# mkln/spamtree

Hardware: AMD Instinct MI355X
Metric: Gibbs iterations/sec + achieved HBM GB/s, n=1e6 grid, 1/2/4/8 MI355X (higher is better)
Workload: dtype f64

## Files before the change

include/spamtree_hip.h:

```cpp
#ifndef SPAMTREE_HIP_H
#define SPAMTREE_HIP_H

#include <stdint.h>

#ifdef __cplusplus
extern "C" {
#endif

#define ST_OK 0
#define ST_ERR_CHOL_ROOT 1
#define ST_ERR_CHOL_REF 2
#define ST_ERR_CHOL_LEAF 3
#define ST_ERR_CHOL_SAMPLE_REF 10
#define ST_ERR_CHOL_SAMPLE_LEAF 11
#define ST_ERR_USAGE (-1)
#define ST_ERR_HIP (-2)
#define ST_ERR_TOPOLOGY (-3)
#define ST_ERR_UNSUPPORTED (-4)

#define ST_MAX_Q 6
#define ST_MAX_ANCESTORS 24

typedef struct st_handle_s *st_handle;

typedef struct st_problem {
  int64_t n_all;
  int32_t d;
  int32_t q;
  int32_t p;
  int32_t n_groups;
  int64_t n_blocks;
  const double *y;
  const double *X;
  const double *coords;
  const int64_t *mv_id;
  const int64_t *res_is_ref;
  const int64_t *block_names;
  const int64_t *block_groups;
  const int64_t *indexing_ptr;
  const int64_t *indexing_idx;
  const int64_t *parents_ptr;
  const int64_t *parents_idx;
  const int64_t *children_ptr;
  const int64_t *children_idx;
} st_problem;

typedef struct st_options {
  int32_t device;
  int32_t reference_quirks;
  int32_t rank;
  int32_t world;
  int32_t force_generic;
  int32_t reserved;
} st_options;

int st_create(const st_problem *pb, const st_options *opt, st_handle *out);
int st_destroy(st_handle h);
const char *st_last_error(st_handle h);

int st_set_w(st_handle h, const double *w);
int st_get_w(st_handle h, double *w);
int st_set_beta(st_handle h, const double *Bcoeff);
int st_set_tausq_inv(st_handle h, const double *tausq_inv);
int st_get_xb(st_handle h, double *xb);

int st_factor(st_handle h, int slot, const double *theta, int ntheta, double *loglik);
int st_factor_enqueue(st_handle h, int slot, const double *theta, int ntheta);
int st_factor_is_async(st_handle h);
int st_factor_finish(st_handle h, double *loglik);
int st_factor_begin(st_handle h, int slot, const double *theta, int ntheta);
int st_factor_ahead_levels(st_handle h);
int st_factor_ahead_enable(st_handle h, int enable);

int st_swap(st_handle h);

int st_sample_w(st_handle h, const double *z, uint64_t seed, uint32_t iter);

int st_loglik_w(st_handle h, int slot, double *loglik);

int st_sample_w_loglik(st_handle h, const double *z, uint64_t seed, uint32_t iter, int slot, double *loglik);
int st_sample_w_loglik_begin(st_handle h, const double *z, uint64_t seed, uint32_t iter, int slot);
int st_sample_w_loglik_end(st_handle h, double *loglik);

int st_predict(st_handle h, int theta_changed);

int st_beta_stats(st_handle h, double *xty);
int st_tausq_stats(st_handle h, double *ssq, int64_t *n_obs_by_q);
int st_xtx(st_handle h, double *xtx);

int st_yhat(st_handle h, const double *noise, uint64_t seed, uint32_t iter, double *yhat);

int st_block_dims(st_handle h, int64_t u, int64_t *m, int64_t *P, int32_t *is_ref, int32_t *n_obs);
int st_get_block(st_handle h, int slot, int64_t u, double *negRiH, double *Ri);
int st_get_comps(st_handle h, int slot, double *logdetCi_comps, double *loglik_w_comps);

int st_algorithmic_bytes(st_handle h, double *out5, double *flops3);
int st_probe_peaks(int device, int64_t bytes, int reps, double *out3);
int st_probe_math(int32_t fn, const double *x, int64_t n, int32_t device, double *out);
#define ST_N_KERNEL_FAMILIES 8
int st_profile_enable(st_handle h, int enable);
int st_profile_get(st_handle h, double *ms_total, int64_t *launches);
int st_profile_levels(st_handle h, int32_t *n_levels, double *ms_by_level, double *bytes_by_level, int32_t cap);
#define ST_KERNEL_GENERIC_LDS 0
#define ST_KERNEL_GENERIC_SCRATCH 1
#define ST_KERNEL_MFMA 2
#define ST_KERNEL_QUAD 3
#define ST_KERNEL_BIGMFMA 4
#define ST_KERNEL_WIDE 5
#define ST_KERNEL_LCHAIN 6
#define ST_KERNEL_LCHAIN_REF 7
int st_level_info(st_handle h, int32_t *n_levels, int32_t *kernel, int32_t *max_m, int32_t *max_P, int32_t *n_blocks, int32_t cap);
#define ST_ROUTE_NONE 0
#define ST_ROUTE_A_SLOTS 3
int st_route_info(st_handle h, int32_t *n_levels, int32_t *phase_a, int32_t *phase_b, int32_t *phase_p, int32_t cap);
const char *st_route_name(int32_t code);
int st_synchronize(st_handle h);
void *st_stream(st_handle h);

int st_cross_covariance_ag10(const double *coords1, const int64_t *mv1, int64_t n1, const double *coords2, const int64_t *mv2,
                             int64_t n2, const double *ai1, const double *ai2, const double *phi_i, const double *thetamv,
                             const double *Dmat, int32_t q, int32_t device, double *out);
int st_summary_reset(st_handle h);
int st_summary_accumulate(st_handle h, uint64_t seed, uint32_t iter);
int st_summary_get(st_handle h, double *w_mean, double *yhat_mean, int64_t *n_accumulated);
int st_summary_reserve(st_handle h, int64_t keep);
int st_summary_quantile(st_handle h, double q, double *w_q, double *yhat_q);

int st_points_set(st_handle h, int64_t n_new, const double *coords, const int64_t *mv, const int64_t *anchor, const double *X);
int st_points_predict(st_handle h, int mode, const double *z, uint64_t seed, uint32_t iter, double *w_new, double *cond_mean,
                      double *cond_var, double *yhat_new);
int st_points_info(st_handle h, int32_t *route, int64_t *n_groups, double *alg_bytes, double *flops);
const char *st_points_route_name(int32_t code);

int st_points_accumulate(st_handle h, uint64_t seed, uint32_t iter, double *w_new, double *cond_mean, double *cond_var, double *yhat_new);
int st_points_summary_reset(st_handle h);
int st_points_summary_reserve(st_handle h, int64_t keep);
int st_points_summary_get(st_handle h, double *mean, double *var, double *w_mean, double *yhat_mean, int64_t *n_accumulated);
int st_points_summary_quantile(st_handle h, double q, double *w_q, double *yhat_q);

int st_simulate(st_handle h, int nd, const double *z, const double *eps, uint64_t seed, uint32_t iter0, double *w_out, double *y_out);
int st_simulate_info(st_handle h, int nd, int32_t *route_mask, double *alg_bytes, double *flops);
const char *st_simulate_route_name(int32_t code);

int st_set_stream(st_handle h, void *stream);

int st_comm_unique_id(void *out, int32_t cap);
int st_comm_init(st_handle h, const void *unique_id);
int st_shard_plan(const st_problem *pb, int32_t world, int64_t *owner , int32_t *cut_level);
int st_shard_plan_opt(const st_problem *pb, const st_options *opt, int32_t world, int64_t *owner , int32_t *cut_level);
int st_shard_info(st_handle h, int32_t *rank, int32_t *world, int32_t *cut_level, int64_t *owned_blocks, int64_t *owned_rows);
int st_factor_local(st_handle h, int slot, const double *theta, int ntheta);
int st_loglik_local(st_handle h, int slot);
int st_mg_pack_comps(st_handle h, int slot, void **dev_ptr, int64_t *len);
int st_mg_finish(st_handle h, double *loglik);
int st_sample_w_local(st_handle h, const double *z, uint64_t seed, uint32_t iter);
int st_mg_top_region(st_handle h, void **dev_ptr, int64_t *len);
int st_sample_w_top(st_handle h);
int st_mg_pack_w(st_handle h, void **dev_ptr, int64_t *len);
int st_mg_unpack_w(st_handle h);
int st_mg_gather_w_pack(st_handle h, void **send_ptr, void **recv_ptr, int64_t *count_per_rank);
int st_mg_gather_w_unpack(st_handle h);
// ... 6 lines not shown
```

spamtree_amd/_lib.py:

```python
import ctypes as C
import os

HERE = os.path.dirname(os.path.abspath(__file__))
LIB_PATH = os.environ.get("SPAMTREE_LIB") or os.path.join(HERE, "libspamtree_hip.so")

c_dp = C.POINTER(C.c_double)
c_ip = C.POINTER(C.c_int64)


class StProblem(C.Structure):
    _fields_ = [("n_all", C.c_int64), ("d", C.c_int32), ("q", C.c_int32), ("p", C.c_int32), ("n_groups", C.c_int32),
                ("n_blocks", C.c_int64), ("y", c_dp), ("X", c_dp), ("coords", c_dp), ("mv_id", c_ip),
                ("res_is_ref", c_ip), ("block_names", c_ip), ("block_groups", c_ip), ("indexing_ptr", c_ip),
                ("indexing_idx", c_ip), ("parents_ptr", c_ip), ("parents_idx", c_ip), ("children_ptr", c_ip),
                ("children_idx", c_ip)]


class StOptions(C.Structure):
    _fields_ = [("device", C.c_int32), ("reference_quirks", C.c_int32), ("rank", C.c_int32), ("world", C.c_int32),
                ("force_generic", C.c_int32), ("reserved", C.c_int32)]


H = C.c_void_p
SIGNATURES = {
    "st_create": (C.c_int, [C.POINTER(StProblem), C.POINTER(StOptions), C.POINTER(H)]),
    "st_destroy": (C.c_int, [H]),
    "st_last_error": (C.c_char_p, [H]),
    "st_set_w": (C.c_int, [H, c_dp]),
    "st_get_w": (C.c_int, [H, c_dp]),
    "st_set_beta": (C.c_int, [H, c_dp]),
    "st_set_tausq_inv": (C.c_int, [H, c_dp]),
    "st_get_xb": (C.c_int, [H, c_dp]),
    "st_factor": (C.c_int, [H, C.c_int, c_dp, C.c_int, c_dp]),
    "st_factor_begin": (C.c_int, [H, C.c_int, c_dp, C.c_int]),
    "st_factor_ahead_levels": (C.c_int, [H]),
    "st_swap": (C.c_int, [H]),
    "st_sample_w": (C.c_int, [H, c_dp, C.c_uint64, C.c_uint32]),
    "st_loglik_w": (C.c_int, [H, C.c_int, c_dp]),
    "st_sample_w_loglik": (C.c_int, [H, c_dp, C.c_uint64, C.c_uint32, C.c_int, c_dp]),
    "st_sample_w_loglik_begin": (C.c_int, [H, c_dp, C.c_uint64, C.c_uint32, C.c_int]),
    "st_sample_w_loglik_end": (C.c_int, [H, c_dp]),
    "st_predict": (C.c_int, [H, C.c_int]),
    "st_beta_stats": (C.c_int, [H, c_dp]),
    "st_tausq_stats": (C.c_int, [H, c_dp, c_ip]),
    "st_xtx": (C.c_int, [H, c_dp]),
    "st_yhat": (C.c_int, [H, c_dp, C.c_uint64, C.c_uint32, c_dp]),
    "st_block_dims": (C.c_int, [H, C.c_int64, c_ip, c_ip, C.POINTER(C.c_int32), C.POINTER(C.c_int32)]),
    "st_get_block": (C.c_int, [H, C.c_int, C.c_int64, c_dp, c_dp]),
    "st_get_comps": (C.c_int, [H, C.c_int, c_dp, c_dp]),
    "st_algorithmic_bytes": (C.c_int, [H, c_dp, c_dp]),
    "st_factor_ahead_enable": (C.c_int, [H, C.c_int]),
    "st_probe_peaks": (C.c_int, [C.c_int, C.c_int64, C.c_int, c_dp]),
    "st_probe_math": (C.c_int, [C.c_int32, c_dp, C.c_int64, C.c_int32, c_dp]),
    "st_profile_enable": (C.c_int, [H, C.c_int]),
    "st_profile_get": (C.c_int, [H, c_dp, c_ip]),
    "st_profile_levels": (C.c_int, [H, C.POINTER(C.c_int32), c_dp, c_dp, C.c_int32]),
    "st_level_info": (C.c_int, [H, C.POINTER(C.c_int32), C.POINTER(C.c_int32), C.POINTER(C.c_int32), C.POINTER(C.c_int32),
                                C.POINTER(C.c_int32), C.c_int32]),
    "st_route_info": (C.c_int, [H, C.POINTER(C.c_int32), C.POINTER(C.c_int32), C.POINTER(C.c_int32), C.POINTER(C.c_int32),
                                C.c_int32]),
    "st_route_name": (C.c_char_p, [C.c_int32]),
    "st_synchronize": (C.c_int, [H]),
    "st_stream": (C.c_void_p, [H]),
    "st_set_stream": (C.c_int, [H, C.c_void_p]),
    "st_shard_plan": (C.c_int, [C.POINTER(StProblem), C.c_int32, c_ip, C.POINTER(C.c_int32)]),
    "st_shard_plan_opt": (C.c_int, [C.POINTER(StProblem), C.POINTER(StOptions), C.c_int32, c_ip, C.POINTER(C.c_int32)]),
    "st_shard_info": (C.c_int, [H, C.POINTER(C.c_int32), C.POINTER(C.c_int32), C.POINTER(C.c_int32), c_ip, c_ip]),
    "st_factor_local": (C.c_int, [H, C.c_int, c_dp, C.c_int]),
    "st_factor_enqueue": (C.c_int, [H, C.c_int, c_dp, C.c_int]),
    "st_factor_finish": (C.c_int, [H, c_dp]),
    "st_factor_is_async": (C.c_int, [H]),
    "st_loglik_local": (C.c_int, [H, C.c_int]),
    "st_mg_pack_comps": (C.c_int, [H, C.c_int, C.POINTER(C.c_void_p), c_ip]),
    "st_mg_finish": (C.c_int, [H, c_dp]),
    "st_sample_w_local": (C.c_int, [H, c_dp, C.c_uint64, C.c_uint32]),
    "st_mg_top_region": (C.c_int, [H, C.POINTER(C.c_void_p), c_ip]),
    "st_sample_w_top": (C.c_int, [H]),
    "st_mg_pack_w": (C.c_int, [H, C.POINTER(C.c_void_p), c_ip]),
    "st_mg_unpack_w": (C.c_int, [H]),
    "st_mg_gather_w_pack": (C.c_int, [H, C.POINTER(C.c_void_p), C.POINTER(C.c_void_p), c_ip]),
    "st_mg_gather_w_unpack": (C.c_int, [H]),
    "st_cross_covariance_ag10": (C.c_int, [c_dp, c_ip, C.c_int64, c_dp, c_ip, C.c_int64, c_dp, c_dp, c_dp, c_dp, c_dp, C.c_int32,
                                           C.c_int32, c_dp]),
    "st_summary_reset": (C.c_int, [H]),
    "st_summary_accumulate": (C.c_int, [H, C.c_uint64, C.c_uint32]),
    "st_summary_get": (C.c_int, [H, c_dp, c_dp, c_ip]),
    "st_summary_reserve": (C.c_int, [H, C.c_int64]),
    "st_summary_quantile": (C.c_int, [H, C.c_double, c_dp, c_dp]),
    "st_comm_unique_id": (C.c_int, [C.c_void_p, C.c_int32]),
    "st_comm_init": (C.c_int, [H, C.c_void_p]),
    "st_points_set": (C.c_int, [H, C.c_int64, c_dp, c_ip, c_ip, c_dp]),
    "st_points_predict": (C.c_int, [H, C.c_int, c_dp, C.c_uint64, C.c_uint32, c_dp, c_dp, c_dp, c_dp]),
    "st_points_info": (C.c_int, [H, C.POINTER(C.c_int32), c_ip, c_dp, c_dp]),
    "st_points_route_name": (C.c_char_p, [C.c_int32]),
    "st_points_accumulate": (C.c_int, [H, C.c_uint64, C.c_uint32, c_dp, c_dp, c_dp, c_dp]),
    "st_points_summary_reset": (C.c_int, [H]),
    "st_points_summary_reserve": (C.c_int, [H, C.c_int64]),
    "st_points_summary_get": (C.c_int, [H, c_dp, c_dp, c_dp, c_dp, c_ip]),
    "st_points_summary_quantile": (C.c_int, [H, C.c_double, c_dp, c_dp]),
    "st_simulate": (C.c_int, [H, C.c_int, c_dp, c_dp, C.c_uint64, C.c_uint32, c_dp, c_dp]),
    "st_simulate_info": (C.c_int, [H, C.c_int, C.POINTER(C.c_int32), c_dp, c_dp]),
    "st_simulate_route_name": (C.c_char_p, [C.c_int32]),
}


class StmFlags(C.Structure):
    _fields_ = [("adapting", C.c_int32), ("sample_beta", C.c_int32), ("sample_tausq", C.c_int32),
                ("sample_theta", C.c_int32), ("sample_w", C.c_int32), ("sample_predicts", C.c_int32)]


SIGNATURES.update({
    "stm_create": (C.c_int, [C.POINTER(StProblem), C.POINTER(StOptions), c_dp, c_dp, c_dp, C.c_int, c_dp, C.c_double,
                             C.c_uint64, C.POINTER(StmFlags), C.POINTER(H)]),
    "stm_init": (C.c_int, [H]),
    "stm_destroy": (C.c_int, [H]),
    "stm_last_error": (C.c_char_p, [H]),
    "stm_handle": (C.c_void_p, [H]),
    "stm_step": (C.c_int, [H, C.c_int]),
    "stm_state": (C.c_int, [H, c_dp, c_dp, c_dp, c_dp, c_dp, c_ip, c_dp]),
    "spamtree_mv_mcmc_c": (C.c_int, [C.POINTER(StProblem), C.POINTER(StOptions), c_dp, c_dp, C.c_int, c_dp, C.c_double,
                                     c_dp, C.c_int, C.c_int, C.c_int, C.c_uint64, C.POINTER(StmFlags), c_dp, c_dp,
# ... 33 lines not shown
```

spamtree_amd/csrc/misc_kernels.hpp:

```cpp
#pragma once
#include "st_device.hpp"

struct LoglikArgs {
  const Blk *blks;
  const int *anc_idx;
  const int *list;
  int nlist;
  const double *panels;
  const double *w;
  double *loglik_c;
  int maxP, maxM;
};

struct LoglikGrpArgs {
  const Blk *blks;
  const int *anc_idx;
  const Grp *grps;
  const int *list;
  int nlist;
  const double *panels;
  const double *w;
  double *loglik_c;
  int maxP;
  const long long *gdesc;
  int gd_stride;
};

#define SUM2_WG 64
#define STATS_WG 1024
struct QtArgs {
  const double *draws;
  long long n;
  int keep, Kpad, R;
  double q;
  double *out;
};

#ifdef ST_DEFS_MISC
__global__ void k_normals(double *z, const long long *dev2model, long long n, unsigned iter, unsigned stream, unsigned long long seed) {
  const long long i = (long long)blockIdx.x * blockDim.x + threadIdx.x;
  if (i < n) z[i] = philox_normal((unsigned long long)dev2model[i], iter, stream, seed);
}


__global__ __launch_bounds__(NT) void k_loglik(LoglikArgs A) {
  extern __shared__ double lds[];
  __shared__ int s_am[MAXJ], s_ao[MAXJ + 1];
  __shared__ long long s_arow[MAXJ];
  __shared__ double s_red[NT / 64];
  const int tid = threadIdx.x, lane = tid & 63, wid = tid >> 6;
  double *wv = lds;
  double *tv = wv + (A.maxP + A.maxM);
  for (int li = blockIdx.x; li < A.nlist; li += gridDim.x) {
    const int b = A.list[li];
    const Blk B = A.blks[b];
    const int m = B.m, P = B.P, J = B.nanc, ld = B.ld;
    __syncthreads();
    if (tid < J) {
      const int a = A.anc_idx[B.anc_ptr + tid];
      s_am[tid] = A.blks[a].m;
      s_arow[tid] = A.blks[a].row0;
    }
    __syncthreads();
    if (tid == 0) {
      int o = 0;
      for (int t = 0; t < J; ++t) { s_ao[t] = o; o += s_am[t]; }
      s_ao[J] = o;
    }
    __syncthreads();
    for (int t = 0; t < J; ++t)
      for (int i = tid; i < s_am[t]; i += NT) wv[s_ao[t] + i] = A.w[s_arow[t] + i];
    for (int i = tid; i < m; i += NT) wv[P + i] = A.w[B.row0 + i];
    __syncthreads();
    const double *N = A.panels + B.panel_off;
    for (int i = wid; i < m; i += NT / 64) {
      double acc = 0.0;
      for (int k = lane; k < P; k += 64) acc += N[(size_t)i * ld + k] * wv[k];
      acc = wave_sum(acc);
      if (lane == 0) tv[i] = acc;
    }
    __syncthreads();
    double part = 0.0;
    for (int i = tid; i < m; i += NT) {
      double acc = tv[i];
      if (B.isref) {
        for (int j = 0; j <= i; ++j) acc += N[(size_t)i * ld + P + j] * wv[P + j];
      } else {
        acc += N[(size_t)i * ld + P] * wv[P + i];
      }
      part += acc * acc;
    }
    const double wcore = block_sum(part, s_red);
    if (tid == 0) A.loglik_c[b] = (double)m * HL2PI - 0.5 * wcore;
  }
}


__global__ __launch_bounds__(NT, 8) void k_loglik_grp(LoglikGrpArgs A) {
  extern __shared__ double lds[];
  __shared__ int s_am[MAXJ], s_ao[MAXJ + 1];
  __shared__ long long s_arow[MAXJ];
  __shared__ long long s_bpan[32], s_brow[32];
  __shared__ int s_bld[32], s_cb[32];
  __shared__ double s_e2[32];
  __shared__ long long s_gd[GD_MAXW];
  const int tid = threadIdx.x, lane = tid & 63, wid = tid >> 6;
  double *wv = lds;
  {
    const long long *gd = A.gdesc + (size_t)A.list[blockIdx.x] * A.gd_stride;
    for (int i = tid; i < A.gd_stride; i += NT) s_gd[i] = gd[i];
  }
  __syncthreads();
  const GdHead B0 = gd_unpack(s_gd, tid, s_am, s_ao, s_arow, nullptr, nullptr, s_bpan, s_brow, s_bld, nullptr);
  const Grp G = {B0.row0, B0.blk0, B0.nblk, B0.M, B0.P};
  const int M = G.M, P = G.P, J = B0.nanc;
  const bool refgrp = B0.isref != 0;
  if (tid >= 128 && tid < 128 + 32) wv[P + tid - 128] = (tid - 128 < M) ? A.w[G.row0 + tid - 128] : 0.0;
  if (tid >= 32 && tid < 64) {
    const int j = tid - 32;
    int bi = 0;
    if (j < M) { const long long r = G.row0 + j; while (bi + 1 < G.nblk && r >= s_gd[8 + 4 * J + 3 * (bi + 1) + 1]) ++bi; }
    s_cb[j] = bi;
  }
  __syncthreads();
  const int rowlen = P + (refgrp ? M : 1);
#pragma unroll 1
  for (int b = 0; b < 2; ++b) {
    double v[4][5];
#pragma unroll
    for (int rr = 0; rr < 4; ++rr) {
      const int j = wid + 4 * (4 * b + rr), jc = min(j, M - 1);
      const int bi = s_cb[jc];
      const double *src = A.panels + s_bpan[bi] + (size_t)(G.row0 + jc - s_brow[bi]) * s_bld[bi];
#pragma unroll
      for (int c = 0; c < 5; ++c) {
        const int k = lane + 64 * c;
        v[rr][c] = (j < M && k < rowlen) ? src[k] : 0.0;
      }
    }
    if (b == 0) {
      for (int k = tid; k < P; k += NT) {
        int t = 0;
        while (t + 1 < J && k >= s_ao[t + 1]) ++t;
        wv[k] = A.w[s_arow[t] + (k - s_ao[t])];
      }
      __syncthreads();
    }
#pragma unroll
    for (int rr = 0; rr < 4; ++rr) {
      const int j = wid + 4 * (4 * b + rr);
      double acc = 0.0;
#pragma unroll
      for (int c = 0; c < 5; ++c) {
        const int k = lane + 64 * c;
        const double wk = k < P ? wv[k] : (refgrp ? (k < rowlen ? wv[k] : 0.0) : wv[P + min(j, 31)]);
        acc += v[rr][c] * wk;
      }
      acc = wave_sum(acc);
      if (lane == 0 && j < 32) s_e2[j] = acc * acc;
    }
  }
  __syncthreads();
  if (tid < G.nblk) {
    double wc = 0.0;
    int cnt = 0;
    for (int j = 0; j < M; ++j)
      if (s_cb[j] == tid) { wc += s_e2[j]; ++cnt; }
    A.loglik_c[G.blk0 + tid] = (double)cnt * HL2PI - 0.5 * wc;
  }
}

__global__ __launch_bounds__(NT) void k_sum2_partial(const double *a, const double *b, int n, double *partial) {
  __shared__ double sa[NT], sb[NT];
  const int chunk = (n + SUM2_WG - 1) / SUM2_WG;
  const int lo = blockIdx.x * chunk, hi = min(n, lo + chunk);
  double xa = 0.0, xb = 0.0;
  for (int i = lo + threadIdx.x; i < hi; i += NT) { xa += a[i]; xb += b[i]; }
  sa[threadIdx.x] = xa; sb[threadIdx.x] = xb;
  __syncthreads();
  for (int s2 = NT / 2; s2 > 0; s2 >>= 1) {
    if ((int)threadIdx.x < s2) { sa[threadIdx.x] += sa[threadIdx.x + s2]; sb[threadIdx.x] += sb[threadIdx.x + s2]; }
    __syncthreads();
  }
  if (threadIdx.x == 0) { partial[2 * blockIdx.x] = sa[0]; partial[2 * blockIdx.x + 1] = sb[0]; }
}
__global__ void k_sum2_final(const double *partial, double *out) {
  if (threadIdx.x < 2) {
    double s2 = 0.0;
    for (int g = 0; g < SUM2_WG; ++g) s2 += partial[2 * g + threadIdx.x];
    out[threadIdx.x] = s2;
  }
}

__global__ void k_xb(const double *X, const int *mv, const double *B, long long n, int p, double *xb) {
  const long long i = (long long)blockIdx.x * blockDim.x + threadIdx.x;
  if (i >= n) return;
  const double *bj = B + (size_t)p * mv[i];
  double acc = 0.0;
  for (int j = 0; j < p; ++j) acc += X[(size_t)j * n + i] * bj[j];
  xb[i] = acc;
}

__global__ __launch_bounds__(NT) void k_stats(const double *X, const double *y, const double *w, const double *xb, const int *mv,
                                               const unsigned char *obs, const long long *partner, long long n, int p, int q,
                                               double *partial) {
  __shared__ double s_red[NT / 64];
  const int nq = p * q + q;
  double acc[QMAX * 8 + QMAX];
  for (int k = 0; k < nq; ++k) acc[k] = 0.0;
  const long long chunk = (n + gridDim.x - 1) / gridDim.x;
  const long long lo = (long long)blockIdx.x * chunk, hi = min(n, lo + chunk);
  for (long long i = lo + threadIdx.x; i < hi; i += NT) {
    if (!obs[i]) continue;
    const int v = mv[i];
    const double rw = y[i] - w[partner[i]];
    for (int j = 0; j < p; ++j) acc[v * p + j] += X[(size_t)j * n + i] * rw;
    const double e = y[i] - xb[i] - w[i];
    acc[p * q + v] += e * e;
  }
  for (int k = 0; k < nq; ++k) {
    const double s = block_sum(acc[k], s_red);
    if (threadIdx.x == 0) partial[(size_t)blockIdx.x * nq + k] = s;
  }
}
__global__ __launch_bounds__(NT) void k_stats_final(const double *partial, int nwg, int nq, double *out) {
  __shared__ double sm[NT];
  const int k = blockIdx.x;
  double s = 0.0;
  for (int g = threadIdx.x; g < nwg; g += NT) s += partial[(size_t)g * nq + k];
  sm[threadIdx.x] = s;
  __syncthreads();
  for (int o = NT / 2; o > 0; o >>= 1) {
    if ((int)threadIdx.x < o) sm[threadIdx.x] += sm[threadIdx.x + o];
    __syncthreads();
  }
  if (threadIdx.x == 0) out[k] = sm[0];
}

__global__ void k_yhat(const double *xb, const double *w, const double *noise, const int *mv, long long n, const double *tsq_inv_q,
                       double *yhat) {
  const long long i = (long long)blockIdx.x * blockDim.x + threadIdx.x;
  if (i < n) yhat[i] = xb[i] + w[i] + noise[i] / sqrt(tsq_inv_q[mv[i]]);
// ... 125 lines not shown
```

spamtree_amd/csrc/sample_kernels.hpp:

```cpp
#pragma once
#include "st_device.hpp"

struct SampleArgs {
  const Blk *blks;
  const int *anc_idx;
  const int *dch_idx;
  const int *list;
  int nlist;
  const double *panels;
  double *w;
  const double *y, *xb, *z;
  const int *mv;
  const unsigned char *obs;
  double *acc;
  int *errflag;
  double *scratch;
  long long scratch_stride;
  int maxP, maxM, maxLd;
  int do_gram;
  int no_fwd;
  int lds_sq;
  double *s0;
  const long long *s0off;
  double tausq_inv[QMAX];
};

struct GramBigArgs {
  const Blk *blks;
  const int *anc_idx, *dch_idx;
  const int *list;
  int nlist;
  const double *panels;
  double *acc;
  double *s0;
  const long long *s0off;
  int no_fwd;
  int mirror;
};

struct SampleFastArgs {
  const Blk *blks;
  const int *anc_idx, *dch_idx;
  const Grp *grps;
  int ngrp;
  const double *panels;
  double *w;
  const double *y, *xb, *z;
  const int *mv;
  double *acc;
  int *errflag;
  const long long *gdesc;
  int gd_stride;
  int ldN, Mr4, Mrows, maxP, av_dbl;
  int do_gram;
  int no_fwd;
  double tausq_inv[QMAX];
  const long long *gdesc_all;
  double *s0;
  const long long *s0off;
  int s0_mode;
};
#define GRAM_DIRECT_MAXCH 4

#ifdef ST_DEFS_SAMPLE

__device__ __forceinline__ void wave_chol_solve_lds(double *S, int ms, double *lcol, double *bv, const double *zg, int m, int *fail, int lane) {
  const int i0 = lane, i1 = 64 + (lane & 15), g1 = lane >> 4;
  const bool r0 = i0 < m, r1 = i1 < m;
  const bool two = m > 64;
  double c0 = r0 ? bv[i0] : 0.0, c1 = r1 ? bv[i1] : 0.0;
  double dr0 = 1.0, dr1 = 1.0;
  bool bad = false;
  for (int j = lane; j < m + 8; j += 64) lcol[j] = 0.0;
  for (int k = 0; k < m; ++k) {
    const double d = S[(size_t)k * ms + k];
    bad = bad || !(d > 0.0);
    double rp = __builtin_amdgcn_rsq(d);
    rp = rp * fma(-0.5 * d * rp, rp, 1.5);
    rp = rp * fma(-0.5 * d * rp, rp, 1.5);
    const bool u0 = r0 && i0 > k, u1 = r1 && i1 > k;
    const double l0 = u0 ? S[(size_t)i0 * ms + k] * rp : 0.0;
    const double l1 = u1 ? S[(size_t)i1 * ms + k] * rp : 0.0;
    const double ck = readlane_f64(k < 64 ? c0 : c1, k & 63);
    const double yk = ck * rp;
    c0 = (i0 == k) ? yk : fma(-l0, yk, c0);
    c1 = (i1 == k) ? yk : fma(-l1, yk, c1);
    dr0 = (i0 == k) ? rp : dr0;
    dr1 = (i1 == k) ? rp : dr1;
    if (u0) { S[(size_t)i0 * ms + k] = l0; lcol[i0] = l0; }
    if (u1 && g1 == 0) { S[(size_t)i1 * ms + k] = l1; lcol[i1] = l1; }
    __builtin_amdgcn_fence(__ATOMIC_ACQ_REL, "wavefront");
    if (r0) {
      double *row = S + (size_t)i0 * ms;
      for (int j0 = k + 1; j0 < m; j0 += 8) {
        double lj[8], a0[8];
#pragma unroll
        for (int q = 0; q < 8; ++q) lj[q] = lcol[j0 + q];
#pragma unroll
        for (int q = 0; q < 8; ++q) a0[q] = row[j0 + q];
#pragma unroll
        for (int q = 0; q < 8; ++q) row[j0 + q] = fma(-l0, lj[q], a0[q]);
      }
    }
    if (two) {
      if (r1) {
        double *row = S + (size_t)i1 * ms;
        for (int j0 = k + 1 + 8 * g1; j0 < m; j0 += 32) {
          double lj[8], a1[8];
#pragma unroll
          for (int q = 0; q < 8; ++q) lj[q] = lcol[j0 + q];
#pragma unroll
          for (int q = 0; q < 8; ++q) a1[q] = row[j0 + q];
#pragma unroll
          for (int q = 0; q < 8; ++q) row[j0 + q] = fma(-l1, lj[q], a1[q]);
        }
      }
    }
    __builtin_amdgcn_fence(__ATOMIC_ACQ_REL, "wavefront");
  }
  if (bad && lane == 0) *fail = 1;
  double t0 = r0 ? c0 + zg[i0] : 0.0, t1 = r1 ? c1 + zg[i1] : 0.0;
  for (int k = m - 1; k >= 0; --k) {
    const double wk = readlane_f64(k < 64 ? t0 : t1, k & 63) * readlane_f64(k < 64 ? dr0 : dr1, k & 63);
    t0 = (i0 == k) ? wk : ((r0 && i0 < k) ? fma(-S[(size_t)k * ms + i0], wk, t0) : t0);
    if (two) t1 = (i1 == k) ? wk : ((r1 && i1 < k) ? fma(-S[(size_t)k * ms + i1], wk, t1) : t1);
  }
  if (r0) bv[i0] = t0;
  if (r1 && g1 == 0) bv[i1] = t1;
}


template <bool BIG, bool NOREF = false>
__global__ __launch_bounds__(NT) void k_sample(SampleArgs A) {
  extern __shared__ double lds[];
  __shared__ int s_am[MAXJ], s_ao[MAXJ + 1];
  __shared__ long long s_arow[MAXJ], s_aoff[MAXJ + 1];
  __shared__ int s_fail;
  __shared__ long long s_choff[16];

  const int tid = threadIdx.x, lane = tid & 63, wid = tid >> 6;
  const int maxP = A.maxP, maxM = A.maxM;
  double *wv = lds;
  double *tv = wv + (maxP + maxM);
// ... 801 lines not shown
    const int t = u >> 1, it = u & 1;
    const bool self = t == J;
    const int ma = self ? M : s_am[t], oa = self ? P : s_ao[t];
    if (it * 16 >= ma) continue;
    const bool wide = ma > 16;
    auto chains = [&](const long long *rowoff, int Mr, d4 (&cq)[2]) __attribute__((always_inline)) {
      const int ns = (Mr + 3) >> 2;
      double b0[8], b1[8];
#pragma unroll
      for (int st = 0; st < 8; ++st) {
        const int r = 4 * st + l4;
        const bool rok = st < ns && r < Mr;
        const double *row = A.panels + rowoff[min(r, 31)] + oa + l15;
        b0[st] = rok ? row[0] : 0.0;
        b1[st] = (rok && wide) ? row[16] : 0.0;
      }
      cq[0] = (d4){0.0, 0.0, 0.0, 0.0}; cq[1] = cq[0];
#pragma unroll
      for (int st = 0; st < 8; ++st)
        if (st < ns) {
          const double ai = it ? b1[st] : b0[st];
          cq[0] = __builtin_amdgcn_mfma_f64_16x16x4f64(ai, b0[st], cq[0], 0, 0, 0);
          if (wide) cq[1] = __builtin_amdgcn_mfma_f64_16x16x4f64(ai, b1[st], cq[1], 0, 0, 0);
        }
    };
    auto store = [&](double *out, const d4 (&v)[2]) __attribute__((always_inline)) {
#pragma unroll
      for (int jt = 0; jt < 2; ++jt) {
        if (jt > 0 && !wide) continue;
#pragma unroll
        for (int r = 0; r < 4; ++r) {
          const int i = it * 16 + l4 + 4 * r, j = jt * 16 + l15;
          if (i < ma && j < ma) out[i * ma + j] = v[jt][r];
        }
      }
    };
    d4 chv[2];
    chv[0] = (d4){0.0, 0.0, 0.0, 0.0}; chv[1] = chv[0];
    for (int cc = 0; cc < nch; ++cc) {
      d4 cch[2];
      chains(s_crow[cc], s_cM[cc], cch);
#pragma unroll
      for (int q = 0; q < 2; ++q)
#pragma unroll
        for (int r = 0; r < 4; ++r) { cch[q][r] += 0.0; chv[q][r] += cch[q][r]; }
      if (self) store(A.acc + s_coff[cc] + B0.acc_len, cch);
    }
    if (!self) {
      d4 c[2];
      chains(s_rowoff, M, c);
#pragma unroll
      for (int q = 0; q < 2; ++q)
#pragma unroll
        for (int r = 0; r < 4; ++r) c[q][r] += chv[q][r];
      store(rec + s_aoff[t], c);
    }
  }
}

template <bool LAT>
__global__ __launch_bounds__(NT, LAT ? 2 : 5) void k_sample_lean(SampleFastArgs A) {
  extern __shared__ double lds[];
  __shared__ int s_am[MAXJ], s_ao[MAXJ + 1];
  __shared__ long long s_arow[MAXJ], s_aoff[MAXJ + 1];
  __shared__ long long s_bpan[32], s_brow[32], s_rowoff[32];
  __shared__ int s_bld[32], s_cb[32];
  __shared__ int s_fail;
  __shared__ long long s_coff[64];
  __shared__ int s_nch;
  __shared__ long long s_gd[GD_MAXW];

  const int tid = threadIdx.x;
  double *wv = lds;
  double *seg = wv + A.maxP + 32;
  double *tv = seg + A.av_dbl + 16, *ev = tv + 32, *bv = ev + 32, *tsq = bv + 32, *yx = tsq + 32, *zc = yx + 32, *rjv = zc + 32;
  double *Rc = rjv + 32;
  double *S = Rc + 32 * CH_LD;

  int gidx = blockIdx.x;
  {
    const int per = A.ngrp >> 3;
    if (gidx < per * 8) gidx = (gidx & 7) * per + (gidx >> 3);
  }
  for (int i = tid; i < A.gd_stride; i += NT) s_gd[i] = A.gdesc[(size_t)gidx * A.gd_stride + i];
  __syncthreads();
  const GdHead B0 = gd_unpack(s_gd, tid, s_am, s_ao, s_arow, nullptr, s_aoff, s_bpan, s_brow, s_bld, s_coff);
  const Grp G = {B0.row0, B0.blk0, B0.nblk, B0.M, B0.P};
  const int M = G.M, P = G.P, J = B0.nanc;
  const bool refgrp = B0.isref != 0;
  if (tid == 0) { s_fail = 0; s_nch = B0.ndch; }
  const long long so = (refgrp && A.s0off && A.s0_mode) ? A.s0off[B0.blk0] : -1;
  const bool s0_load = so >= 0 && A.s0_mode == 2;
  double xq[28], x2[28], ch2[4], s0v[3], smv[4];
  const int k2 = tid - 64;
  const int nch2 = A.no_fwd ? 0 : B0.ndch;
  if constexpr (LAT) {
    double t_ = 0.0, y_ = 0.0, xb_ = 0.0, z_ = 0.0, r_ = 0.0;
    int mv_ = 0;
    const bool rowthr = tid >= 32 && tid < 64 && tid - 32 < M;
    if (tid >= 32 && tid < 64) {
      const int j = tid - 32;
      int bi = 0;
      long long ro = 0;
      if (j < M) {
        const long long r = G.row0 + j;
        mv_ = A.mv[r]; y_ = A.y[r]; xb_ = A.xb[r]; z_ = A.z[r];
        const long long *gb = s_gd + 8 + 4 * J;
        while (bi + 1 < G.nblk && r >= gb[3 * (bi + 1) + 1]) ++bi;
        ro = gb[3 * bi] + (r - gb[3 * bi + 1]) * gb[3 * bi + 2];
        if (!refgrp) r_ = A.panels[ro + P];
      }
      s_cb[j] = bi; s_rowoff[j] = ro;
    }
    lds_barrier();
    double wreg = 0.0;
    int wk = -1;
    if (tid < P) {
      int t = 0;
      while (t + 1 < J && tid >= s_ao[t + 1]) ++t;
      wk = tid; wreg = A.w[s_arow[t] + (tid - s_ao[t])];
    }
    double rireg[3];
#pragma unroll
    for (int e = 0; e < 3; ++e) {
      const int idx = tid + NT * e, i = idx / M, j = idx - i * M;
      rireg[e] = (refgrp && idx < M * M && j <= i) ? A.panels[s_rowoff[i] + P + j] : 0.0;
    }
    {
      const int idx = tid, mj = M * J;
      const int ii = mj > 0 ? min(idx, mj - 1) : 0, r = J ? ii / J : 0, t = J ? ii - r * J : 0;
      const int ma = J ? s_am[t] : 0;
      const double *row = A.panels + s_rowoff[r] + (J ? s_ao[t] : 0);
#pragma unroll
      for (int jj = 0; jj < 28; ++jj) xq[jj] = (idx < mj && jj < ma) ? row[jj] : 0.0;
    }
#pragma unroll
    for (int cc = 0; cc < 4; ++cc)
      smv[cc] = (refgrp && tid < M && cc < B0.ndch) ? A.acc[s_coff[min(cc, max(B0.ndch - 1, 0))] + B0.acc_len + M * M + tid] : 0.0;
    if (k2 >= 0 && k2 < P) {
      int t = 0;
      while (t + 1 < J && k2 >= s_ao[t + 1]) ++t;
      const int ma = s_am[t], i = k2 - s_ao[t];
#pragma unroll
      for (int cc = 0; cc < 4; ++cc) ch2[cc] = (cc < nch2) ? A.acc[s_coff[min(cc, max(nch2 - 1, 0))] + s_aoff[t] + ma * ma + i] : 0.0;
#pragma unroll
      for (int rr = 0; rr < 28; ++rr) x2[rr] = (rr < M) ? A.panels[s_rowoff[min(rr, M - 1)] + k2] : 0.0;
    }
#pragma unroll
    for (int e = 0; e < 3; ++e) {
      const int idx = tid + NT * e, i = idx / M, j = idx - i * M;
      s0v[e] = (s0_load && idx < M * M && j <= i) ? A.s0[so + idx] : 0.0;
    }
    if (rowthr) t_ = A.tausq_inv[mv_];
    if (tid >= 32 && tid < 64) { const int j = tid - 32; tsq[j] = t_; yx[j] = y_ - xb_; zc[j] = z_; rjv[j] = r_; }
    if (wk >= 0) wv[wk] = wreg;
    for (int k = NT + tid; k < P; k += NT) {
      int t = 0;
      while (t + 1 < J && k >= s_ao[t + 1]) ++t;
      wv[k] = A.w[s_arow[t] + (k - s_ao[t])];
    }
    if (refgrp) {
#pragma unroll
      for (int e = 0; e < 3; ++e) {
        const int idx = tid + NT * e, i = idx / M, j = idx - i * M;
        if (idx < M * M) Rc[i * CH_LD + j] = rireg[e];
      }
      for (int idx = 3 * NT + tid; idx < M * M; idx += NT) {
        const int i = idx / M, j = idx - i * M;
        Rc[i * CH_LD + j] = (j <= i) ? A.panels[s_rowoff[i] + P + j] : 0.0;
      }
    }
    __syncthreads();
  } else {
  if (tid >= 32 && tid < 64) {
    const int j = tid - 32;
    double t_ = 0.0, y_ = 0.0, z_ = 0.0, r_ = 0.0;
    int bi = 0;
    long long ro = 0;
    if (j < M) {
      const long long r = G.row0 + j;
      t_ = A.tausq_inv[A.mv[r]]; y_ = A.y[r] - A.xb[r]; z_ = A.z[r];
      const long long *gb = s_gd + 8 + 4 * J;
      while (bi + 1 < G.nblk && r >= gb[3 * (bi + 1) + 1]) ++bi;
      ro = gb[3 * bi] + (r - gb[3 * bi + 1]) * gb[3 * bi + 2];
      if (!refgrp) r_ = A.panels[ro + P];
    }
    tsq[j] = t_; yx[j] = y_; zc[j] = z_; rjv[j] = r_; s_cb[j] = bi; s_rowoff[j] = ro;
  }
  __syncthreads();
  for (int k = tid; k < P; k += NT) {
    int t = 0;
    while (t + 1 < J && k >= s_ao[t + 1]) ++t;
    wv[k] = A.w[s_arow[t] + (k - s_ao[t])];
  }
  if (refgrp) {
    for (int idx = tid; idx < M * M; idx += NT) {
      const int i = idx / M, j = idx - i * M;
      Rc[i * CH_LD + j] = (j <= i) ? A.panels[s_rowoff[i] + P + j] : 0.0;
    }
  }
  __syncthreads();
  }
  for (int idx = tid; idx < M * J; idx += NT) {
    const int r = idx / J, t = idx - r * J;
    const int ma = s_am[t], oa = s_ao[t];
    const double *row = A.panels + s_rowoff[r] + oa;
    const double *wa = wv + oa;
    double a = 0.0;
    if (LAT && idx == tid && ma <= 28) {
#pragma unroll
      for (int jj = 0; jj < 28; ++jj) a += xq[jj] * ((jj < ma) ? wa[jj] : 0.0);
    } else
    for (int j0 = 0; j0 < ma; j0 += 16) {
      double x[16];
#pragma unroll
      for (int jj = 0; jj < 16; ++jj) x[jj] = (j0 + jj < ma) ? row[j0 + jj] : 0.0;
#pragma unroll
      for (int jj = 0; jj < 16; ++jj) a += x[jj] * ((j0 + jj < ma) ? wa[j0 + jj] : 0.0);
    }
    seg[t * 32 + r] = a;
  }
  __syncthreads();
  if (tid < M) {
    double a = 0.0;
    for (int t = 0; t < J; ++t) a += seg[t * 32 + tid];
    tv[tid] = a;
  }
  __syncthreads();
  if (refgrp) {
    for (int idx = tid; idx < M * M; idx += NT) {
      const int i = idx / M, j = idx - i * M;
      double a = 0.0;
      if (j <= i) {
        if (s0_load) a = (LAT && idx < 3 * NT) ? (idx < NT ? s0v[0] : (idx < 2 * NT ? s0v[1] : s0v[2])) : A.s0[so + idx];
        else {
          double ch[4];
          for (int c0 = 0; c0 < s_nch; c0 += 4) {
#pragma unroll
            for (int cc = 0; cc < 4; ++cc) ch[cc] = (c0 + cc < s_nch) ? A.acc[s_coff[min(c0 + cc, s_nch - 1)] + B0.acc_len + idx] : 0.0;
            if (c0 == 0) for (int k = i; k < M; ++k) a += Rc[k * CH_LD + i] * Rc[k * CH_LD + j];
#pragma unroll
            for (int cc = 0; cc < 4; ++cc) a += ch[cc];
          }
          if (s_nch == 0) for (int k = i; k < M; ++k) a += Rc[k * CH_LD + i] * Rc[k * CH_LD + j];
          if (so >= 0) A.s0[so + idx] = a;
        }
        if (i == j) a += tsq[i];
      }
      S[i * CH_LD + j] = a;
    }
    if (tid < M) {
      const int i = tid;
      double a = 0.0;
      for (int k = i; k < M; ++k) a -= Rc[k * CH_LD + i] * tv[k];
      double ch[4];
      for (int c0 = 0; c0 < s_nch; c0 += 4) {
#pragma unroll
        for (int cc = 0; cc < 4; ++cc)
          ch[cc] = (LAT && c0 == 0) ? smv[cc] : ((c0 + cc < s_nch) ? A.acc[s_coff[min(c0 + cc, s_nch - 1)] + B0.acc_len + M * M + i] : 0.0);
#pragma unroll
        for (int cc = 0; cc < 4; ++cc) a += ch[cc];
      }
      bv[i] = a + tsq[i] * yx[i];
    }
    double *pub = seg + 32 * J;
    if (M <= 27) {
      __syncthreads();
      if (tid < 64) wave_chol_solve<27>(S, bv, zc, wv + P, M, &s_fail, tid);
      __syncthreads();
    } else {
      team_chol_eliminate<5, NT>(S, S, M, M, pub, &s_fail, tid);
      if (tid < M) {
        double a = zc[tid];
        for (int j = 0; j <= tid; ++j) a += S[tid * CH_LD + j] * bv[j];
        ev[tid] = a;
      }
      __syncthreads();
      if (tid < M) {
        double a = 0.0;
        for (int i = tid; i < M; ++i) a += S[i * CH_LD + tid] * ev[i];
        wv[P + tid] = a;
      }
      __syncthreads();
    }
    if (tid < M) {
      const int i = tid;
      A.w[G.row0 + i] = wv[P + i];
      double a = tv[i];
      for (int j = 0; j <= i; ++j) a += Rc[i * CH_LD + j] * wv[P + j];
      ev[i] = a;
    }
  } else {
    if (tid < M) {
      const int j = tid;
      const double rj = rjv[j];
      const double sig = rj * rj + tsq[j];
      if (!(sig > 0.0)) s_fail = 1;
      const double mu = -rj * tv[j] + tsq[j] * yx[j];
      const double c = 1.0 / sqrt(sig);
      const double wj = c * c * mu + c * zc[j];
      A.w[G.row0 + j] = wj;
      ev[j] = rj * wj + tv[j];
    }
  }
  __syncthreads();
  for (int idx = tid; idx < J * 32; idx += NT) {
    const int r = idx & 31;
    seg[idx] = (r < M) ? ev[r] - seg[idx] : 0.0;
  }
  __syncthreads();
  double *rec = A.acc + B0.acc_off;
  const int kfirst = LAT ? (tid >= 64 ? k2 : NT - 64 + tid) : tid;
  for (int k = kfirst; k < P; k += NT) {
    int t = 0;
    while (t + 1 < J && k >= s_ao[t + 1]) ++t;
    const int ma = s_am[t], i = k - s_ao[t];
    const double *avt = seg + t * 32;
    const bool held = LAT && tid >= 64 && k == k2 && M <= 28;
    double ch[4];
    const int nch = A.no_fwd ? 0 : s_nch;
#pragma unroll
    for (int cc = 0; cc < 4; ++cc) ch[cc] = held ? ch2[cc] : ((cc < nch) ? A.acc[s_coff[min(cc, max(nch - 1, 0))] + s_aoff[t] + ma * ma + i] : 0.0);
    double a = 0.0;
    if (held) {
#pragma unroll
      for (int rr = 0; rr < 28; ++rr) a -= x2[rr] * avt[min(rr, 31)];
    } else
    for (int r0 = 0; r0 < M; r0 += 8) {
      double x[8];
#pragma unroll
      for (int rr = 0; rr < 8; ++rr) x[rr] = (r0 + rr < M) ? A.panels[s_rowoff[min(r0 + rr, M - 1)] + k] : 0.0;
#pragma unroll
      for (int rr = 0; rr < 8; ++rr) a -= x[rr] * avt[min(r0 + rr, 31)];
    }
#pragma unroll
    for (int cc = 0; cc < 4; ++cc) a += ch[cc];
    for (int c0 = 4; c0 < nch; c0 += 4) {
#pragma unroll
      for (int cc = 0; cc < 4; ++cc) ch[cc] = (c0 + cc < nch) ? A.acc[s_coff[min(c0 + cc, nch - 1)] + s_aoff[t] + ma * ma + i] : 0.0;
#pragma unroll
      for (int cc = 0; cc < 4; ++cc) a += ch[cc];
    }
    rec[s_aoff[t] + ma * ma + i] = a;
  }
  if (tid == 0 && s_fail) atomicMin(A.errflag, B0.level * 16 + (refgrp ? 10 : 11));
}
template __global__ void k_sample_lean<false>(SampleFastArgs);
template __global__ void k_sample_lean<true>(SampleFastArgs);

#define WSYNC() asm volatile("s_waitcnt lgkmcnt(0)" ::: "memory")
__global__ __launch_bounds__(NT, 3) void k_sample_wave(SampleFastArgs A) {
  extern __shared__ double lds[];
  __shared__ int s_failw[NT / 64];
  const int tid = threadIdx.x, lane = tid & 63, wid = tid >> 6;
  const int gidx = blockIdx.x * (NT / 64) + wid;
  if (gidx >= A.ngrp) return;
  double *base = lds + (size_t)wid * A.ldN;
  long long *s_gd = (long long *)base;
  double *wv = base + A.gd_stride;
  double *seg = wv + A.maxP + 32;
  double *tv = seg + A.av_dbl, *ev = tv + 32;
  double *Rc = ev + 32;
  if (lane == 0) s_failw[wid] = 0;
  for (int i = lane; i < A.gd_stride; i += 64) s_gd[i] = A.gdesc[(size_t)gidx * A.gd_stride + i];
  WSYNC();
  auto slo = [](long long v) { return __builtin_amdgcn_readfirstlane((int)(v & 0xffffffffLL)); };
  auto shi = [](long long v) { return __builtin_amdgcn_readfirstlane((int)(v >> 32)); };
  auto sll = [&](long long v) { return ((long long)shi(v) << 32) | (unsigned int)slo(v); };
  const long long row0 = sll(s_gd[0]), acc_off = sll(s_gd[1]);
  const int M = slo(s_gd[2]), P = shi(s_gd[2]), J = slo(s_gd[3]), level = shi(s_gd[4]);
  const int nch = slo(s_gd[5]), acc_len = shi(s_gd[5]);
  const long long *gb = s_gd + 8 + 4 * J;
  const long long bpan = sll(gb[0]);
  const int bld = (int)sll(gb[2]);
  const long long *coff = gb + 3;
  auto am_of = [&](int t) { return (int)(s_gd[8 + 4 * t] & 0xffffffffLL); };
  auto ao_of = [&](int t) { return (int)(s_gd[8 + 4 * t] >> 32); };
  const bool row = lane < M;
  const int li = min(lane, 31);
  double tsq = 0.0, yx = 0.0, zc = 0.0;
  if (row) { const long long r = row0 + lane; tsq = A.tausq_inv[A.mv[r]]; yx = A.y[r] - A.xb[r]; zc = A.z[r]; }
  for (int k = lane; k < P; k += 64) {
    int t = 0;
    for (int j = 1; j < J; ++j) t += k >= ao_of(j) ? 1 : 0;
    wv[k] = A.w[s_gd[8 + 4 * t + 1] + (k - ao_of(t))];
  }
  const int PS = P | 1;
  const int RG = min(4, (A.Mrows * CH_LD) / PS);
  if (RG >= 1) {
    constexpr int NRI = (27 * 27 + 63) / 64;
    double rireg[NRI];
#pragma unroll
    for (int q = 0; q < NRI; ++q) {
      const int idx = lane + 64 * q, i = idx / M, j = idx - i * M;
      rireg[q] = (idx < M * M && j <= i) ? A.panels[bpan + (size_t)i * bld + P + j] : 0.0;
    }
    double *stg = Rc;
    for (int r0 = 0; r0 < M; r0 += RG) {
      for (int c0 = 0; 64 * c0 < P; c0 += 4) {
        double x[4][4];
#pragma unroll
        for (int rr = 0; rr < 4; ++rr)
#pragma unroll
          for (int c = 0; c < 4; ++c) {
            const int k = lane + 64 * (c0 + c);
            x[rr][c] = (rr < RG && r0 + rr < M && k < P) ? A.panels[bpan + (size_t)(r0 + rr) * bld + k] : 0.0;
          }
#pragma unroll
        for (int rr = 0; rr < 4; ++rr)
#pragma unroll
          for (int c = 0; c < 4; ++c) {
            const int k = lane + 64 * (c0 + c);
            if (rr < RG && k < P) stg[rr * PS + k] = x[rr][c];
          }
      }
      WSYNC();
      if (lane < RG * J) {
        const int rr = lane / J, t = lane - rr * J, r = r0 + rr;
        if (r < M) {
          const int ma = am_of(t), oa = ao_of(t);
          const double *srow = stg + rr * PS + oa;
          const double *wa = wv + oa;
          double a = 0.0;
          for (int j = 0; j < ma; ++j) a += srow[j] * wa[j];
          seg[t * 32 + r] = a;
        }
      }
    }
    WSYNC();
#pragma unroll
    for (int q = 0; q < NRI; ++q) {
      const int idx = lane + 64 * q, i = idx / M, j = idx - i * M;
      if (idx < M * M) Rc[i * CH_LD + j] = rireg[q];
    }
    WSYNC();
  } else {
  for (int idx = lane; idx < M * M; idx += 64) {
    const int i = idx / M, j = idx - i * M;
    Rc[i * CH_LD + j] = (j <= i) ? A.panels[bpan + (size_t)i * bld + P + j] : 0.0;
  }
  WSYNC();
  for (int idx = lane; idx < M * J; idx += 64) {
    const int r = idx / J, t = idx - r * J;
    const int ma = am_of(t), oa = ao_of(t);
    const double *prow = A.panels + bpan + (size_t)r * bld + oa;
    const double *wa = wv + oa;
    double a = 0.0;
    for (int j0 = 0; j0 < ma; j0 += 16) {
      double x[16];
#pragma unroll
      for (int jj = 0; jj < 16; ++jj) x[jj] = (j0 + jj < ma) ? prow[j0 + jj] : 0.0;
#pragma unroll
      for (int jj = 0; jj < 16; ++jj) a += x[jj] * ((j0 + jj < ma) ? wa[j0 + jj] : 0.0);
    }
    seg[t * 32 + r] = a;
  }
  WSYNC();
  }
  double tvi = 0.0;
  if (row) { for (int t = 0; t < J; ++t) tvi += seg[t * 32 + lane]; tv[lane] = tvi; }
  WSYNC();
  double a[27];
#pragma unroll
  for (int j = 0; j < 27; ++j) a[j] = 0.0;
  double bv = 0.0;
  const long long so = (A.s0off && A.s0_mode) ? A.s0off[slo(s_gd[6])] : -1;
  if (so >= 0 && A.s0_mode == 2) {
    const double *sp = A.s0 + so + (size_t)li * M;
#pragma unroll
    for (int j = 0; j < 27; ++j) a[j] = (row && j <= lane) ? sp[j] : 0.0;
    for (int k = 0; k < M; ++k) bv -= Rc[k * CH_LD + li] * tv[k];
    for (int c = 0; c < nch; ++c) bv += row ? A.acc[coff[c] + acc_len + M * M + li] : 0.0;
  } else {
    for (int k = 0; k < M; ++k) {
      const double rk = Rc[k * CH_LD + li];
      bv -= rk * tv[k];
#pragma unroll
      for (int j = 0; j < 27; ++j) a[j] += rk * Rc[k * CH_LD + j];
    }
    for (int c = 0; c < nch; ++c) {
      const double *rc = A.acc + coff[c] + acc_len;
      double ch[27];
#pragma unroll
      for (int j = 0; j < 27; ++j) ch[j] = (row && j <= lane) ? rc[li * M + j] : 0.0;
      const double cv = row ? rc[M * M + li] : 0.0;
#pragma unroll
      for (int j = 0; j < 27; ++j) a[j] += ch[j];
      bv += cv;
    }
    if (so >= 0 && row) {
      double *sp = A.s0 + so + (size_t)li * M;
#pragma unroll
      for (int j = 0; j < 27; ++j) if (j <= lane) sp[j] = a[j];
    }
  }
#pragma unroll
  for (int j = 0; j < 27; ++j) {
    if (j == lane) a[j] += tsq;
    a[j] = (row && j <= lane) ? a[j] : (j == lane ? 1.0 : 0.0);
  }
  bv = row ? bv + tsq * yx : 0.0;
  const double wnew = wave_chol_solve_core<27>(a, bv, zc, M, &s_failw[wid], lane);
  if (row) { A.w[row0 + lane] = wnew; wv[P + lane] = wnew; }
  WSYNC();
  if (row) {
    double e = tvi;
    for (int j = 0; j <= lane; ++j) e += Rc[lane * CH_LD + j] * wv[P + j];
    ev[lane] = e;
  }
  WSYNC();
  for (int idx = lane; idx < J * 32; idx += 64) {
    const int r = idx & 31;
    seg[idx] = (r < M) ? ev[r] - seg[idx] : 0.0;
  }
  WSYNC();
  double *rec = A.acc + acc_off;
  const int nfw = A.no_fwd ? 0 : nch;
  for (int k = lane; k < P; k += 64) {
    int t = 0;
    for (int j = 1; j < J; ++j) t += k >= ao_of(j) ? 1 : 0;
    const int ma = am_of(t), i = k - ao_of(t);
    const long long aoff = s_gd[8 + 4 * t + 3];
    const double *avt = seg + t * 32;
    double ch[4];
#pragma unroll
    for (int cc = 0; cc < 4; ++cc) ch[cc] = (cc < nfw) ? A.acc[coff[min(cc, max(nfw - 1, 0))] + aoff + ma * ma + i] : 0.0;
    double acc = 0.0;
    for (int r0 = 0; r0 < M; r0 += 8) {
      double x[8];
#pragma unroll
      for (int rr = 0; rr < 8; ++rr) x[rr] = (r0 + rr < M) ? A.panels[bpan + (size_t)min(r0 + rr, M - 1) * bld + k] : 0.0;
#pragma unroll
      for (int rr = 0; rr < 8; ++rr) acc -= x[rr] * avt[min(r0 + rr, 31)];
    }
#pragma unroll
    for (int cc = 0; cc < 4; ++cc) acc += ch[cc];
// ... 368 lines not shown
```

spamtree_amd/csrc/spamtree_hip.hip:

```cpp

#include "st_device.hpp"
#include "factor_generic.hpp"
#include "factor_mfma.hpp"
#include "chol_blocked.hpp"
#include "factor_quad.hpp"
#include "factor_big.hpp"
#include "factor_wide.hpp"
#include "factor_lchain.hpp"
#include "sample_kernels.hpp"
#include "misc_kernels.hpp"
#include "predict_points.hpp"
#include "simulate_kernels.hpp"

static thread_local std::string g_create_error;
struct st_handle_s;
static void points_free(st_handle_s *h);

template <typename T>
struct DevBuf {
  T *p = nullptr;
  size_t n = 0;
  hipError_t alloc(size_t count) {
    n = count;
    if (count == 0) { p = nullptr; return hipSuccess; }
    return hipMalloc((void **)&p, count * sizeof(T));
  }
  hipError_t upload(const std::vector<T> &v) {
    hipError_t e = alloc(v.size());
    if (e != hipSuccess || v.empty()) return e;
    return hipMemcpy(p, v.data(), v.size() * sizeof(T), hipMemcpyHostToDevice);
  }
  void free() { if (p) (void)hipFree(p); p = nullptr; n = 0; }
};

struct LevelInfo {
  int first = 0, count = 0;
  int isref = 1;
  int maxP = 0, maxM = 0, maxMa = 0, maxLd = 0;
  bool big_factor = false, big_sample = false, sample_sq = false;
  size_t lds_factor = 0, lds_sample = 0, lds_loglik = 0;
  double alg_bytes_A = 0, alg_bytes_B = 0, alg_bytes_C = 0, alg_bytes_msg = 0;
  double flops_A = 0, flops_B = 0, flops_C = 0;
  bool fast = false;
  int grp_first = 0, grp_count = 0, Pm4 = 0, ldKV = 2, ldS = 2, SRm = 1, stage_dbl = 0;
  size_t lds_fast = 0;
  int ldN = 2, Mr4 = 4, Mrows = 1, av_dbl = 224, maxJ = 0;
  size_t lds_sfast = 0, lds_slean = 0;
  bool bigmfma = false;
  int wide_first = 0, wide_count = 0, wide_maxN = 0;
  size_t lds_wide = 0;
  int bm_ldS = 0;
  size_t lds_bigmfma = 0;
  int lchain = 0;
  bool lchain_ref = false;
  size_t lds_ref_finish = 0;
  int rf_first = 0;
  int lc_first = 0, lc_count = 0;
  int quad_first = 0, quad_count = 0, qown_lo = 0, qown_n = 0, q_ldS = 0, q_nkx = 0;
  long long vl_off = -1;
  size_t lds_quad = 0;
  int own_lo = 0, own_n = 0, gown_lo = 0, gown_n = 0;
};

enum RouteCode : int {
  R_NONE = ST_ROUTE_NONE,
  R_MARGINAL_INVCHOL_WAVE, R_MARGINAL_INVCHOL,
  R_FACTOR_LDS, R_FACTOR_SCRATCH, R_PREDICT_LDS, R_PREDICT_SCRATCH,
  R_QUAD32_REF_WCH, R_QUAD32_REF, R_QUAD32_LEAF, R_QUAD38_REF_WCH, R_QUAD38_REF, R_QUAD38_LEAF,
  R_QUAD44_REF_WCH, R_QUAD44_REF, R_QUAD44_LEAF, R_QUAD50_REF_WCH, R_QUAD50_REF, R_QUAD50_LEAF,
  R_FACTOR_MFMA, R_LCHAIN96, R_LCHAIN136, R_REF_FINISH, R_LCHAIN_SCALARS, R_FACTOR_WIDE, R_BIGMFMA3, R_BIGMFMA4, R_BIGMFMA5,
  R_GRAM, R_GRAM_DIRECT, R_GRAM_BIG,
  R_SAMPLE_MFMA, R_LEAF_SEG4, R_LEAF_SEG6, R_SAMPLE_LEAF, R_SAMPLE_WAVE, R_SAMPLE_LEAN_LAT, R_SAMPLE_LEAN,
  R_SAMPLE_BIG_REF, R_SAMPLE_LEAF_WIDE, R_SAMPLE_BIG_LEAF, R_SAMPLE_SMALL,
  R_COUNT
};
static const char *const k_route_names[R_COUNT] = {
  "",
  "k_marginal_invchol_wave", "k_marginal_invchol",
  "k_factor<false, MODE_FACTOR>", "k_factor<true, MODE_FACTOR>", "k_factor<false, MODE_PREDICT>", "k_factor<true, MODE_PREDICT>",
  "k_factor_quad<4, 32, 8, true, true>", "k_factor_quad<4, 32, 8, true, false>", "k_factor_quad<4, 32, 8, false, true>",
  "k_factor_quad<4, 38, 10, true, true>", "k_factor_quad<4, 38, 10, true, false>", "k_factor_quad<4, 38, 10, false, true>",
  "k_factor_quad<4, 44, 11, true, true>", "k_factor_quad<4, 44, 11, true, false>", "k_factor_quad<4, 44, 11, false, true>",
  "k_factor_quad<4, 50, 13, true, true>", "k_factor_quad<4, 50, 13, true, false>", "k_factor_quad<4, 50, 13, false, true>",
  "k_factor_mfma", "k_factor_lchain<96>", "k_factor_lchain<136>", "k_factor_ref_finish", "k_lchain_scalars", "k_factor_wide<WG_JT>",
  "k_factor_bigmfma<3, 5, 34>", "k_factor_bigmfma<4, 5, 34>", "k_factor_bigmfma<5, 3, 24>",
  "k_gram", "k_gram_direct", "k_gram_big",
  "k_sample_mfma", "k_sample_leaf_seg<4>", "k_sample_leaf_seg<6>", "k_sample_leaf", "k_sample_wave", "k_sample_lean<true>",
  "k_sample_lean<false>", "k_sample<true, false>", "k_sample_leaf_wide", "k_sample<true, true>", "k_sample<false>",
};

struct Switches {
  int wide = 1, split_gram = 1, sample_wave = 1;
  bool lchain = true, lchain_ref = true, gram_big = true, gram_direct = true, sample_lean = true, sample_lat = true,
       leaf_seg = true, leaf_wide = true, async_top = true;
  int lchain_ref_min = 1;
  int factor_gen = 3;
  int quad_units = 0;
  int quad_min = -1;
};

static Switches read_switches() {
  auto level = [](const char *name) {
    const char *e = getenv(name);
    return (e && e[0] == '0') ? 0 : ((e && e[0] == '2') ? 2 : 1);
  };
  Switches s;
  s.wide = level("SPAMTREE_WIDE"); s.split_gram = level("SPAMTREE_SPLIT_GRAM"); s.sample_wave = level("SPAMTREE_SAMPLE_WAVE");
  s.lchain = level("SPAMTREE_LCHAIN"); s.lchain_ref = level("SPAMTREE_LCHAIN_REF"); s.gram_big = level("SPAMTREE_GRAM_BIG");
  s.gram_direct = level("SPAMTREE_GRAM_DIRECT"); s.sample_lean = level("SPAMTREE_SAMPLE_LEAN"); s.sample_lat = level("SPAMTREE_SAMPLE_LAT");
  s.leaf_seg = level("SPAMTREE_LEAF_SEG"); s.leaf_wide = level("SPAMTREE_LEAF_WIDE"); s.async_top = level("SPAMTREE_ASYNC_TOP");
  const char *e;
  if ((e = getenv("SPAMTREE_LCHAIN_REF_MIN"))) s.lchain_ref_min = atoi(e);
  if ((e = getenv("SPAMTREE_FACTOR_KERNEL")) && e[0] == '1') s.factor_gen = 1;
  if ((e = getenv("SPAMTREE_QUAD_UNITS"))) s.quad_units = atoi(e);
  if ((e = getenv("SPAMTREE_QUAD_MIN"))) s.quad_min = std::max(atoi(e), 0);
  return s;
}

struct st_handle_s {
  std::string err;
  int device = 0;
  hipStream_t stream = nullptr;
  int quirks = 1, force_generic = 0;
  Switches sw;
  long long n_all = 0, n_blocks = 0;
  int q = 1, p = 1, d = 2, n_groups = 0, n_actual_groups = 0;
  long long n_obs = 0;
  size_t lds_limit = 65536;
  int sm_count = 256;

  std::vector<long long> dev2model, model2dev;
  std::vector<int> blk_model2dev;
  std::vector<Blk> blks;
  std::vector<int> anc_idx, dch_idx, lvl_list, pred_list, all_obs_list;
  std::vector<Grp> grps;
  DevBuf<Grp> d_grps;
  std::vector<Quad> quads;
  DevBuf<Quad> d_quads;
  std::vector<WideGrp> wgrps;
  DevBuf<WideGrp> d_wgrps;
  std::vector<LcSlab> lcslabs;
  DevBuf<LcSlab> d_lcslabs;
  std::vector<long long> rfvoff;
  DevBuf<long long> d_rfvoff;
  DevBuf<double> d_vscr;
  size_t vscr_need = 0;
  DevBuf<double> d_lcrow;
  DevBuf<double> d_s0;
  DevBuf<long long> d_s0off;
  bool c_pending = false;
  int c_rc = 0; double c_ll = 0.0;
  std::vector<long long> gdesc;
  DevBuf<long long> d_gdesc;
  int gd_stride = 8;
  int quad_nu = 4;
  int rank = 0, world = 1, cut = 0;
  std::vector<int> blk_owner;
  std::vector<int> own_obs_list;
  DevBuf<int> d_ownobs;
  std::vector<int> own_grp_list, own_obs_slow;
  DevBuf<int> d_owngrp, d_ownslow;
  DevBuf<unsigned char> d_rowmask, d_blkmask;
  DevBuf<double> d_comm;
  DevBuf<double> d_gather;
  DevBuf<int> d_gidx;
  int gather_cnt = 1;
  DevBuf<double> d_gerr;
  hipStream_t stream2 = nullptr;
  hipEvent_t ev_top = nullptr, ev_main = nullptr;
  DevBuf<int> d_err2, d_toplist;
  int n_toplist = 0, g_top = 0;
  bool async_top = false, top_pending = false, prof_suspend = false, async_top_off = false;
  hipEvent_t ev_stats = nullptr;
  bool stats_on_stream2 = false;
  bool stats_prefetched = false;
  int top_phys = -1;
  std::vector<double> top_theta;
  long long top_off = 0, top_len = 0;
  std::vector<std::pair<long long, long long>> top_zero;
  bool ext_stream = false;
  DevBuf<double> d_sum_w, d_sum_yhat;
  long long n_summary = 0;
  DevBuf<double> d_draws_w, d_draws_yhat;
  long long draws_cap = 0, n_draws = 0;
  int gram_direct_level = -1;
  bool stats_valid = false;
  bool host_stats_valid = false;
  std::vector<double> host_stats;
  double *pin = nullptr;
  double *pin_up = nullptr;
  int pin_up_slot = 0, pin_up_len = 0;
  hipEvent_t ev_up[2] = {nullptr, nullptr};
  bool factor_open = false; int factor_open_slot = 0;
  std::vector<double> top_theta_open;
  hipEvent_t ev_factor = nullptr;
  std::vector<char> s0_valid;
  bool gram_valid = false;
  bool cache_gram = true;
  bool defer_leaf = false;
  bool leaf_pending[2] = {false, false};
  CovPar leaf_cp[2];
  DevBuf<double> d_vleaf;
  bool limited = false;
  std::vector<int> twin_list;
  DevBuf<int> d_twin;
  int twin_maxM = 1;
  ncclComm_t comm = nullptr;
  std::vector<LevelInfo> levels;
  std::vector<int> route_a, route_b;
  int route_p = R_NONE;
  LevelInfo pred_info;
  int pred_grp_first = 0, pred_grp_count = 0, pred_quad_first = 0, pred_quad_count = 0, pred_nkx = 0;
  size_t pred_lds = 0;
  std::vector<double> xtx;
  std::vector<long long> n_obs_q;
  struct PointSet *pts = nullptr;
  DevBuf<double> d_simz, d_sime, d_simw, d_simy;
  DevBuf<int> d_rowblk;
  int sim_cap = 0;
  std::vector<SimLevel> sim_levels;

  DevBuf<double> d_cx, d_cy, d_y, d_X, d_w, d_xb, d_z, d_B, d_panels[2], d_acc, d_logdet[2], d_loglik[2], d_scalars, d_partial,
      d_stats, d_scratch, d_tmp_n, d_tsq;
  DevBuf<int> d_mv, d_anc, d_dch, d_lvl, d_pred, d_allobs, d_err;
  DevBuf<unsigned char> d_obs;
  DevBuf<long long> d_dev2model, d_partner;
  DevBuf<Blk> d_blks;
  size_t panel_total = 0, acc_total = 0;
  long long scratch_stride = 0;
  int scratch_wgs = 0;
  int slot_map[2] = {0, 1};
  double tausq_inv[QMAX];
  std::vector<double> theta[2];
  bool z_valid = false;

  int prof = 0;
  double prof_ms[ST_N_KERNEL_FAMILIES] = {0};
  long long prof_n[ST_N_KERNEL_FAMILIES] = {0};
  std::vector<double> prof_level_ms;
  std::vector<long long> prof_level_n;
  struct ProfRec { hipEvent_t a, b; int fam, level, count; };
  std::vector<ProfRec> prof_pending;
  std::vector<hipEvent_t> ev_free;
};

#define HCHK(h, call)                                                                                         \
  do {                                                                                                        \
    hipError_t e_ = (call);                                                                                   \
    if (e_ != hipSuccess) {                                                                                   \
      (h)->err = std::string(#call) + ": " + hipGetErrorString(e_);                                           \
      return ST_ERR_HIP;                                                                                      \
    }                                                                                                         \
  } while (0)

static int fail_create(st_handle_s *h, int code, const std::string &msg) {
  g_create_error = msg;
  if (h) {
    st_destroy(h);
  }
  return code;
}

static hipEvent_t prof_event(st_handle_s *h) {
  if (!h->ev_free.empty()) { hipEvent_t e = h->ev_free.back(); h->ev_free.pop_back(); return e; }
  hipEvent_t e = nullptr;
  (void)hipEventCreate(&e);
  return e;
}
static void prof_harvest(st_handle_s *h) {
  for (auto &r : h->prof_pending) {
    float ms = 0.f;
    if (hipEventSynchronize(r.b) == hipSuccess && hipEventElapsedTime(&ms, r.a, r.b) == hipSuccess) {
      h->prof_ms[r.fam] += ms;
      h->prof_n[r.fam] += r.count;
      if (r.level >= 0 && r.level < (int)h->prof_level_ms.size()) { h->prof_level_ms[r.level] += ms; h->prof_level_n[r.level] += r.count > 0; }
    }
    h->ev_free.push_back(r.a);
    h->ev_free.push_back(r.b);
  }
  h->prof_pending.clear();
}
struct ProfScope {
  st_handle_s *h;
  st_handle_s::ProfRec r;
  hipStream_t st;
  ProfScope(st_handle_s *h_, int fam, int level = -1, int count = 1, hipStream_t st_ = nullptr) : h(h_), st(st_ ? st_ : h_->stream) {
    r.fam = fam; r.level = level; r.count = count; r.a = r.b = nullptr;
    const bool on = level == -2 ? (h->prof == 2 && !h->prof_suspend) : h->prof == 1;
    if (on) { r.a = prof_event(h); r.b = prof_event(h); (void)hipEventRecord(r.a, st); }
  }
  ~ProfScope() {
    if (r.a && r.b) {
      (void)hipEventRecord(r.b, st);
      h->prof_pending.push_back(r);
      if (h->prof_pending.size() > 8192) prof_harvest(h);
    }
  }
};

static void invalidate_stats(st_handle_s *h) {
  if (h->stats_on_stream2) {
    (void)hipSetDevice(h->device);
    (void)hipStreamWaitEvent(h->stream, h->ev_stats, 0);
    h->stats_on_stream2 = false;
  }
  h->stats_valid = false; h->host_stats_valid = false;
}

static size_t lds_factor_bytes(int maxP, int maxM, int maxMa, int SR, bool big) {
  size_t dbl = (size_t)3 * (maxP + maxM) + 3 * (size_t)maxM + (size_t)SR * maxP;
  size_t bytes = dbl * 8 + (size_t)((maxP + maxM + 1) & ~1) * 4;
  if (!big) bytes += ((size_t)2 * maxP * maxM + (size_t)maxMa * maxM + (size_t)2 * maxM * maxM) * 8;
  return bytes + 64;
}
static size_t scratch_factor_doubles(int maxP, int maxM, int maxMa) {
  return (size_t)2 * maxP * maxM + (size_t)maxMa * maxM + (size_t)2 * maxM * maxM;
}
static size_t lds_sample_sq_bytes(int maxM) { return ((size_t)maxM * ((maxM + 7) | 1) + maxM + 16) * 8; }
static size_t lds_sample_bytes(int maxP, int maxM, int maxLd, bool big) {
  size_t dbl = (size_t)(maxP + maxM) + 4 * (size_t)maxM + (size_t)MAXJ * maxM;
  if (!big) dbl += (size_t)maxM * maxLd + (size_t)maxM * maxM;
  return dbl * 8 + 64;
}
static size_t lds_loglik_bytes(int maxP, int maxM) { return ((size_t)maxP + 2 * (size_t)maxM) * 8 + 64; }

extern "C" const char *st_last_error(st_handle h) { return h ? h->err.c_str() : g_create_error.c_str(); }
extern "C" void st_set_create_error(const char *msg) { g_create_error = msg ? msg : ""; }

extern "C" int st_destroy(st_handle h) {
  if (!h) return ST_OK;
  (void)hipSetDevice(h->device);
  h->d_cx.free(); h->d_cy.free(); h->d_y.free(); h->d_X.free(); h->d_w.free(); h->d_xb.free(); h->d_z.free(); h->d_B.free();
  h->d_panels[0].free(); h->d_panels[1].free(); h->d_acc.free();
  for (int s = 0; s < 2; ++s) { h->d_logdet[s].free(); h->d_loglik[s].free(); }
  h->d_scalars.free(); h->d_partial.free(); h->d_stats.free(); h->d_scratch.free(); h->d_tmp_n.free(); h->d_tsq.free();
  h->d_mv.free(); h->d_anc.free(); h->d_dch.free(); h->d_lvl.free(); h->d_pred.free(); h->d_allobs.free(); h->d_err.free();
  h->d_twin.free(); h->d_wgrps.free(); h->d_lcslabs.free(); h->d_lcrow.free(); h->d_rfvoff.free(); h->d_vscr.free(); h->d_vleaf.free(); h->d_s0.free(); h->d_s0off.free(); h->d_obs.free(); h->d_dev2model.free(); h->d_partner.free(); h->d_blks.free(); h->d_grps.free(); h->d_quads.free(); h->d_gdesc.free();
  h->d_ownobs.free(); h->d_owngrp.free(); h->d_ownslow.free(); h->d_rowmask.free(); h->d_blkmask.free(); h->d_comm.free(); h->d_gather.free(); h->d_gidx.free(); h->d_gerr.free(); h->d_err2.free(); h->d_toplist.free();
  if (h->ev_top) (void)hipEventDestroy(h->ev_top);
  if (h->ev_main) (void)hipEventDestroy(h->ev_main);
  if (h->ev_stats) (void)hipEventDestroy(h->ev_stats);
  if (h->stream2) (void)hipStreamDestroy(h->stream2); h->d_sum_w.free(); h->d_sum_yhat.free(); h->d_draws_w.free(); h->d_draws_yhat.free();
  prof_harvest(h);
  for (auto e : h->ev_free) (void)hipEventDestroy(e);
  if (h->comm) (void)ncclCommDestroy(h->comm);
  if (h->pin) (void)hipHostFree(h->pin);
  if (h->pin_up) (void)hipHostFree(h->pin_up);
  for (int i = 0; i < 2; ++i) if (h->ev_up[i]) (void)hipEventDestroy(h->ev_up[i]);
  if (h->ev_factor) (void)hipEventDestroy(h->ev_factor);
  points_free(h);
  h->d_simz.free(); h->d_sime.free(); h->d_simw.free(); h->d_simy.free(); h->d_rowblk.free();
  if (h->stream && !h->ext_stream) (void)hipStreamDestroy(h->stream);
  delete h;
  return ST_OK;
}

static int create_impl(const st_problem *pb, const st_options *opt, st_handle *out, bool plan_only, int64_t *owner_out, int32_t *cut_out);

extern "C" int st_create(const st_problem *pb, const st_options *opt, st_handle *out) {
  return create_impl(pb, opt, out, false, nullptr, nullptr);
}

extern "C" int st_shard_plan(const st_problem *pb, int32_t world, int64_t *owner, int32_t *cut_level) {
  st_options opt = {0, 1, 0, world, 0, 0};
  st_handle dummy = nullptr;
  return create_impl(pb, &opt, &dummy, true, owner, cut_level);
}
extern "C" int st_shard_plan_opt(const st_problem *pb, const st_options *opt_in, int32_t world, int64_t *owner, int32_t *cut_level) {
  st_options opt = {0, 1, 0, world, 0, 0};
  if (opt_in) { opt.reference_quirks = opt_in->reference_quirks; opt.force_generic = opt_in->force_generic; opt.reserved = opt_in->reserved; }
  st_handle dummy = nullptr;
  return create_impl(pb, &opt, &dummy, true, owner, cut_level);
}

static int create_impl(const st_problem *pb, const st_options *opt, st_handle *out, bool plan_only, int64_t *owner_out, int32_t *cut_out) {
  if (!pb || !out) { g_create_error = "st_create: null argument"; return ST_ERR_USAGE; }
  *out = nullptr;
  if (pb->d != 2) { g_create_error = "only d=2 is reachable from spamtree() (R/spamtree_fit.R:58-60)"; return ST_ERR_UNSUPPORTED; }
  if (pb->q < 1 || pb->q > QMAX) { g_create_error = "q out of range"; return ST_ERR_UNSUPPORTED; }
  if (pb->p < 1 || pb->p > 8) { g_create_error = "p must be in 1..8"; return ST_ERR_UNSUPPORTED; }
  if (opt && (opt->world < 1 || opt->rank < 0 || opt->rank >= opt->world || opt->world > 64)) { g_create_error = "bad rank/world"; return ST_ERR_USAGE; }
  if (pb->n_all > 0 && !pb->coords) { g_create_error = "st_create: coords is NULL"; return ST_ERR_USAGE; }
  for (int64_t i = 0; i < 2 * pb->n_all; ++i)
    if (!std::isfinite(pb->coords[i])) {
      g_create_error = "st_create: coordinates must be finite (row " + std::to_string(i % pb->n_all) + ")";
      return ST_ERR_USAGE;
    }
  st_handle_s *h = new st_handle_s();
  h->rank = opt ? opt->rank : 0;
  h->world = opt ? opt->world : 1;
  h->device = opt ? opt->device : 0;
  h->quirks = opt ? opt->reference_quirks : 1;
  h->force_generic = opt ? opt->force_generic : 0;
  h->cache_gram = !(opt && (opt->reserved & 1));
  h->limited = opt && (opt->reserved & 2);
  h->defer_leaf = !(opt && (opt->reserved & 4));
  h->sw = read_switches();
  const long long n = pb->n_all, nb = pb->n_blocks;
  h->n_all = n; h->n_blocks = nb; h->q = pb->q; h->p = pb->p; h->d = pb->d; h->n_groups = pb->n_groups;
  for (int j = 0; j < QMAX; ++j) h->tausq_inv[j] = 1.0;

  std::vector<int> m_of(nb), obs_of(nb, 0), grp_of(nb);
  std::vector<long long> labels(pb->block_groups, pb->block_groups + nb);
  std::sort(labels.begin(), labels.end());
  labels.erase(std::unique(labels.begin(), labels.end()), labels.end());
  if ((int)labels.size() > pb->n_groups) return fail_create(h, ST_ERR_TOPOLOGY, "more levels in block_groups than entries in res_is_ref");
  std::vector<char> row_seen(n, 0);
  for (long long u = 0; u < nb; ++u) {
    m_of[u] = (int)(pb->indexing_ptr[u + 1] - pb->indexing_ptr[u]);
    grp_of[u] = (int)(std::lower_bound(labels.begin(), labels.end(), pb->block_groups[u]) - labels.begin());
    for (long long k = pb->indexing_ptr[u]; k < pb->indexing_ptr[u + 1]; ++k) {
      const long long r = pb->indexing_idx[k];
      if (r < 0 || r >= n || row_seen[r]) return fail_create(h, ST_ERR_TOPOLOGY, "indexing is not a partition of the rows");
      row_seen[r] = 1;
      if (std::isfinite(pb->y[r])) obs_of[u]++;
    }
  }
  for (long long r = 0; r < n; ++r)
    if (!row_seen[r]) return fail_create(h, ST_ERR_TOPOLOGY, "row without a block");
  const int G = (int)labels.size();
// ... 610 lines not shown
    auto pack = [](long long lo, long long hi) { return (lo & 0xffffffffLL) | (hi << 32); };
    std::vector<long long> blk2grp((size_t)nb, -1);
    for (size_t g = 0; g < h->grps.size(); ++g)
      for (int b = 0; b < h->grps[g].nblk; ++b) blk2grp[h->grps[g].blk0 + b] = (long long)g;
    for (size_t g = 0; g < h->grps.size(); ++g) {
      const Grp &G = h->grps[g];
      const Blk &B0 = h->blks[G.blk0];
      long long *w = h->gdesc.data() + g * (size_t)stride;
      const int nch = std::min(B0.ndch, 64);
      w[0] = G.row0; w[1] = B0.acc_off; w[2] = pack(G.M, G.P); w[3] = pack(B0.nanc, G.nblk); w[4] = pack(B0.isref, B0.level);
      w[5] = pack(nch, h->limited ? 0 : B0.acc_len); w[6] = pack(G.blk0, 0);
      long long ao = 0, aoff = 0;
      for (int t = 0; t < B0.nanc; ++t) {
        const Blk &Ba = h->blks[h->anc_idx[B0.anc_ptr + t]];
        long long *a = w + 8 + 4 * t;
        a[0] = pack(Ba.m, ao); a[1] = Ba.row0; a[2] = Ba.chain_off; a[3] = aoff;
        ao += Ba.m; aoff += (long long)Ba.m * Ba.m + Ba.m;
      }
      w[7] = aoff;
      for (int b = 0; b < G.nblk; ++b) {
        const Blk &Bb = h->blks[G.blk0 + b];
        long long *q = w + 8 + 4 * B0.nanc + 3 * b;
        q[0] = Bb.panel_off; q[1] = Bb.row0; q[2] = Bb.ld;
      }
      for (int c = 0; c < nch; ++c) w[8 + 4 * B0.nanc + 3 * G.nblk + c] = h->blks[h->dch_idx[B0.dch_ptr + c]].acc_off;
      for (int c = 0; c < nch; ++c) w[8 + 4 * B0.nanc + 3 * G.nblk + nch + c] = blk2grp[h->dch_idx[B0.dch_ptr + c]];
    }
    h->gram_direct_level = -1;
    {
      const int gl = n_actual - 1, gp = n_actual - 2;
      if (h->sw.gram_direct && gp >= 0 && !h->limited && h->levels[gl].fast && !h->levels[gl].isref && h->levels[gp].fast && h->levels[gp].isref &&
          h->levels[gl].maxM <= 32 && h->levels[gl].maxP <= 255) {
        bool ok = true;
        const LevelInfo &Lp = h->levels[gp], &Ll = h->levels[gl];
        for (int k = 0; k < Lp.grp_count && ok; ++k) {
          const Grp &G = h->grps[Lp.grp_first + k];
          const Blk &B0 = h->blks[G.blk0];
          if (G.nblk != 1 || B0.ndch > GRAM_DIRECT_MAXCH) ok = false;
          for (int c = 0; c < B0.ndch && ok; ++c) {
            const long long cg = blk2grp[h->dch_idx[B0.dch_ptr + c]];
            if (cg < Ll.grp_first || cg >= Ll.grp_first + Ll.grp_count || h->grps[cg].M > 32) ok = false;
          }
        }
        for (int k = 0; k < Ll.grp_count && ok; ++k) {
          const Grp &G = h->grps[Ll.grp_first + k];
          for (int b = 0; b < G.nblk && ok; ++b) {
            const Blk &Bl = h->blks[G.blk0 + b];
            if (Bl.nanc == 0 || h->blks[h->anc_idx[Bl.anc_ptr + Bl.nanc - 1]].level != gp) ok = false;
          }
        }
        if (ok) h->gram_direct_level = gp;
      }
    }
    CCHK(h->d_gdesc.upload(h->gdesc));
  }
  { std::vector<Quad> g = h->quads; if (g.empty()) g.push_back(Quad{0, 0, 0, 0}); CCHK(h->d_quads.upload(g)); }
  { std::vector<WideGrp> g = h->wgrps; if (g.empty()) g.push_back(WideGrp{0, 0}); CCHK(h->d_wgrps.upload(g)); }
  if (!h->lcslabs.empty()) { CCHK(h->d_lcslabs.upload(h->lcslabs)); CCHK(h->d_lcrow.alloc((size_t)2 * h->n_all)); }
  if (!h->rfvoff.empty()) { CCHK(h->d_rfvoff.upload(h->rfvoff)); CCHK(h->d_vscr.alloc(h->vscr_need + (size_t)2 * RF_BUFD)); }
  {
    std::vector<long long> s0off((size_t)(nb > 0 ? nb : 1), -1);
    size_t tot = 0;
    for (int g = 0; g < n_actual; ++g) {
      const LevelInfo &L = h->levels[g];
      if (!L.isref || !(L.big_sample || L.fast)) continue;
      for (int k = 0; k < L.count; ++k) {
        const int b = h->lvl_list[L.first + k];
        s0off[b] = (long long)tot;
        tot += (size_t)h->blks[b].m * h->blks[b].m;
      }
    }
    CCHK(h->d_s0off.upload(s0off));
    CCHK(h->d_s0.alloc(std::max(tot, (size_t)1)));
  }
  { std::vector<int> a = h->pred_list; if (a.empty()) a.push_back(0); CCHK(h->d_pred.upload(a)); }
  CCHK(h->d_allobs.upload(h->all_obs_list));
  { std::vector<int> a = h->own_obs_list; if (a.empty()) a.push_back(0); CCHK(h->d_ownobs.upload(a)); }
  for (int g = 0; g < n_actual; ++g) {
    const LevelInfo &L = h->levels[g];
    if (L.fast) for (int k = 0; k < L.gown_n; ++k) h->own_grp_list.push_back(L.grp_first + L.gown_lo + k);
  }
  for (int b : h->own_obs_list) if (!h->levels[h->blks[b].level].fast) h->own_obs_slow.push_back(b);
  { std::vector<int> a = h->own_grp_list; if (a.empty()) a.push_back(0); CCHK(h->d_owngrp.upload(a)); }
  { std::vector<int> a = h->own_obs_slow; if (a.empty()) a.push_back(0); CCHK(h->d_ownslow.upload(a)); }
  CCHK(h->d_rowmask.upload(rowmask)); CCHK(h->d_blkmask.upload(blkmask));
  CCHK(h->d_comm.alloc((size_t)2 * nb + 64));
  {
    std::vector<std::vector<int>> rows_of(h->world);
    for (int i = 0; i < nb; ++i) {
      const int o = h->blk_owner[i];
      if (o < 0) continue;
      const Blk &B = h->blks[i];
      for (int r2 = 0; r2 < B.m; ++r2) rows_of[o].push_back((int)(B.row0 + r2));
    }
    size_t mx = 0;
    for (auto &v : rows_of) mx = std::max(mx, v.size());
    h->gather_cnt = (int)mx + 1;
    std::vector<int> gi((size_t)h->world * h->gather_cnt, -1);
    for (int r = 0; r < h->world; ++r)
      for (size_t i2 = 0; i2 < rows_of[r].size(); ++i2) gi[(size_t)r * h->gather_cnt + i2] = rows_of[r][i2];
    CCHK(h->d_gidx.upload(gi));
    CCHK(h->d_gather.alloc(gi.size()));
    CCHK(h->d_gerr.alloc(64));
  }
  CCHK(h->d_w.alloc(n)); CCHK(h->d_xb.alloc(n)); CCHK(h->d_z.alloc(n)); CCHK(h->d_tmp_n.alloc(n + 64));
  CCHK(hipMemset(h->d_w.p, 0, n * sizeof(double)));
  CCHK(hipMemset(h->d_xb.p, 0, n * sizeof(double)));
  CCHK(hipMemset(h->d_z.p, 0, n * sizeof(double)));
  CCHK(h->d_B.alloc((size_t)pb->p * pb->q));
  CCHK(h->d_tsq.alloc(QMAX));
  for (int s = 0; s < 2; ++s) {
    CCHK(h->d_panels[s].alloc(h->panel_total + 128));
    CCHK(hipMemset(h->d_panels[s].p, 0, (h->panel_total + 128) * sizeof(double)));
    CCHK(h->d_logdet[s].alloc(nb)); CCHK(h->d_loglik[s].alloc(nb));
    CCHK(hipMemset(h->d_logdet[s].p, 0, nb * sizeof(double)));
    CCHK(hipMemset(h->d_loglik[s].p, 0, nb * sizeof(double)));
  }
  CCHK(h->d_acc.alloc(std::max<size_t>(h->acc_total, 1)));
  CCHK(hipMemset(h->d_acc.p, 0, std::max<size_t>(h->acc_total, 1) * sizeof(double)));
  CCHK(h->d_scalars.alloc(8 + 2 * SUM2_WG));
  CCHK(h->d_err.alloc(2));
  CCHK(h->d_partial.alloc((size_t)STATS_WG * (pb->p * pb->q + pb->q)));
  CCHK(h->d_stats.alloc((size_t)pb->p * pb->q + pb->q));
  {
    size_t need = 0;
    auto upd = [&](const LevelInfo &L) {
      if (L.big_factor || L.bigmfma) need = std::max(need, scratch_factor_doubles(L.maxP, L.maxM, L.maxMa));
      if (L.wide_count > 0) need = std::max(need, (size_t)2 * L.maxP * L.wide_maxN + (size_t)L.maxMa * L.wide_maxN);
      if (L.big_sample) need = std::max(need, (size_t)L.maxM * L.maxM);
    };
    for (auto &L : h->levels) upd(L);
    if (!h->pred_list.empty()) upd(h->pred_info);
    if (need > 0) {
      h->scratch_wgs = h->sm_count * 4;
      h->scratch_stride = (long long)((need + 15) & ~(size_t)15);
      CCHK(h->d_scratch.alloc((size_t)h->scratch_wgs * h->scratch_stride));
    }
  }
  const int lim = (int)h->lds_limit;
  (void)hipFuncSetAttribute((const void *)k_factor<false, MODE_FACTOR>, hipFuncAttributeMaxDynamicSharedMemorySize, lim);
  (void)hipFuncSetAttribute((const void *)k_factor<true, MODE_FACTOR>, hipFuncAttributeMaxDynamicSharedMemorySize, lim);
  (void)hipFuncSetAttribute((const void *)k_factor<false, MODE_PREDICT>, hipFuncAttributeMaxDynamicSharedMemorySize, lim);
  (void)hipFuncSetAttribute((const void *)k_factor<true, MODE_PREDICT>, hipFuncAttributeMaxDynamicSharedMemorySize, lim);
  (void)hipFuncSetAttribute((const void *)k_sample<false>, hipFuncAttributeMaxDynamicSharedMemorySize, lim);
  (void)hipFuncSetAttribute((const void *)k_sample<true>, hipFuncAttributeMaxDynamicSharedMemorySize, lim);
  (void)hipFuncSetAttribute((const void *)k_sample<true, true>, hipFuncAttributeMaxDynamicSharedMemorySize, lim);
  (void)hipFuncSetAttribute((const void *)k_loglik, hipFuncAttributeMaxDynamicSharedMemorySize, lim);
  (void)hipFuncSetAttribute((const void *)k_factor_mfma, hipFuncAttributeMaxDynamicSharedMemorySize, lim);
  (void)hipFuncSetAttribute((const void *)k_factor_wide<WG_JT>, hipFuncAttributeMaxDynamicSharedMemorySize, lim);
  {
    hipFuncAttributes fa;
    size_t st96 = 16 * 1024, st136 = 16 * 1024;
    bool ok96 = false, ok136 = false;
    if (hipFuncGetAttributes(&fa, (const void *)k_factor_lchain<96>) == hipSuccess) { st96 = fa.sharedSizeBytes; ok96 = fa.localSizeBytes == 0; }
    if (hipFuncGetAttributes(&fa, (const void *)k_factor_lchain<136>) == hipSuccess) { st136 = fa.sharedSizeBytes; ok136 = fa.localSizeBytes == 0; }
    for (auto &L : h->levels) {
      if (!L.lchain) continue;
      const size_t need = lc_dyn_doubles(L.lchain) * 8 + (L.lchain == 96 ? st96 : st136);
      if (need > 160 * 1024 || !(L.lchain == 96 ? ok96 : ok136)) { L.lchain = 0; L.lchain_ref = false; }
      if (L.lchain_ref) {
        L.lds_ref_finish = rf_lds_bytes(L.maxM);
        if (L.lds_ref_finish > h->lds_limit) { L.lchain = 0; L.lchain_ref = false; }
      }
    }
    (void)hipFuncSetAttribute((const void *)k_factor_ref_finish, hipFuncAttributeMaxDynamicSharedMemorySize, lim);
    (void)hipFuncSetAttribute((const void *)k_factor_lchain<96>, hipFuncAttributeMaxDynamicSharedMemorySize, (int)(lc_dyn_doubles(96) * 8));
// ... 5 lines not shown
  (void)hipFuncSetAttribute((const void *)k_sample_mfma, hipFuncAttributeMaxDynamicSharedMemorySize, lim);
  (void)hipFuncSetAttribute((const void *)k_sample_wave, hipFuncAttributeMaxDynamicSharedMemorySize, lim);
  (void)hipFuncSetAttribute((const void *)k_marginal_invchol, hipFuncAttributeMaxDynamicSharedMemorySize, lim);
  (void)hipFuncSetAttribute((const void *)k_marginal_invchol_wave, hipFuncAttributeMaxDynamicSharedMemorySize, lim);
  {
    const void *fq = (const void *)k_factor_quad<4, 50, 13, false, true>;
    hipFuncAttributes fa;
    size_t stat = 24 * 1024;
    if (hipFuncGetAttributes(&fa, fq) == hipSuccess) stat = fa.sharedSizeBytes;
    {
      const void *fr = (const void *)k_factor_quad<4, 50, 13, true, true>;
      if (hipFuncGetAttributes(&fa, fr) == hipSuccess) stat = std::max(stat, (size_t)fa.sharedSizeBytes);
      const void *ft = (const void *)k_factor_quad<4, 50, 13, true, false>;
      if (hipFuncGetAttributes(&fa, ft) == hipSuccess) stat = std::max(stat, (size_t)fa.sharedSizeBytes);
    }
    for (auto &L : h->levels) {
      if (L.q_nkx == 0) continue;
      if (L.lds_quad + stat > 160 * 1024) L.q_nkx = 0;
    }
    if (h->pred_nkx && h->pred_lds + stat > 160 * 1024) h->pred_nkx = 0;
#define QATTR(NU_, NKX_, NKT_)                                                                                                       \
  (void)hipFuncSetAttribute((const void *)k_factor_quad<NU_, NKX_, NKT_, true, true>, hipFuncAttributeMaxDynamicSharedMemorySize, 160 * 1024 - (int)stat); \
  (void)hipFuncSetAttribute((const void *)k_factor_quad<NU_, NKX_, NKT_, true, false>, hipFuncAttributeMaxDynamicSharedMemorySize, 160 * 1024 - (int)stat); \
  (void)hipFuncSetAttribute((const void *)k_factor_quad<NU_, NKX_, NKT_, false, true>, hipFuncAttributeMaxDynamicSharedMemorySize, 160 * 1024 - (int)stat)
    QATTR(4, 50, 13); QATTR(4, 44, 11); QATTR(4, 38, 10); QATTR(4, 32, 8);
#undef QATTR
    size_t vl = 0;
    for (auto &L : h->levels) {
      L.vl_off = -1;
      if (!h->defer_leaf || h->world > 1 || h->limited || h->sw.factor_gen != 3 || !L.fast || L.isref || L.q_nkx == 0 || L.qown_n == 0) continue;
      L.vl_off = (long long)vl;
      vl += (size_t)L.qown_n * quad_vtiles(L.q_nkx) * (2 * h->quad_nu) * 256;
    }
    if (vl) CCHK(h->d_vleaf.alloc(vl));
  }
  {
    h->g_top = 0;
    bool all_fast = !h->limited && !h->force_generic;
    for (int g = 0; g < n_actual; ++g) all_fast = all_fast && h->levels[g].fast;
    if (all_fast) {
      while (h->g_top < n_actual && !(h->sw.factor_gen == 3 && h->levels[h->g_top].q_nkx > 0)) ++h->g_top;
      if (h->g_top >= n_actual) h->g_top = 0;
    }
    h->async_top = h->g_top > 0 && h->sw.async_top;
    std::vector<int> tl;
    for (int b : h->own_obs_list) if (h->blks[b].level < h->g_top) tl.push_back(b);
    h->n_toplist = (int)tl.size();
    if (tl.empty()) tl.push_back(0);
    CCHK(h->d_toplist.upload(tl));
    CCHK(h->d_err2.alloc(2));
    if (h->async_top) {
      CCHK(hipStreamCreateWithFlags(&h->stream2, hipStreamNonBlocking));
      CCHK(hipEventCreateWithFlags(&h->ev_top, hipEventDisableTiming));
      CCHK(hipEventCreateWithFlags(&h->ev_main, hipEventDisableTiming));
      CCHK(hipEventCreateWithFlags(&h->ev_stats, hipEventDisableTiming));
    }
  }
  (void)hipGetLastError();
#undef CCHK
  h->s0_valid.assign((size_t)std::max(n_actual, 1), 0);
  h->prof_level_ms.assign(2 * n_actual, 0.0);
  h->prof_level_n.assign(2 * n_actual, 0);
  *out = h;
  return ST_OK;
}

static int upload_rows(st_handle h, const double *src, double *dst) {
  std::vector<double> tmp(h->n_all);
  for (long long i = 0; i < h->n_all; ++i) tmp[i] = src[h->dev2model[i]];
  HCHK(h, hipMemcpyAsync(dst, tmp.data(), h->n_all * sizeof(double), hipMemcpyHostToDevice, h->stream));
  HCHK(h, hipStreamSynchronize(h->stream));
  return ST_OK;
}
static int download_rows(st_handle h, const double *src, double *dst) {
  std::vector<double> tmp(h->n_all);
  HCHK(h, hipMemcpyAsync(tmp.data(), src, h->n_all * sizeof(double), hipMemcpyDeviceToHost, h->stream));
  HCHK(h, hipStreamSynchronize(h->stream));
  for (long long i = 0; i < h->n_all; ++i) dst[h->dev2model[i]] = tmp[i];
  return ST_OK;
}

extern "C" int st_set_w(st_handle h, const double *w) {
  if (!h || !w) return ST_ERR_USAGE;
  invalidate_stats(h);
  HCHK(h, hipSetDevice(h->device));
  return upload_rows(h, w, h->d_w.p);
}
extern "C" int st_get_w(st_handle h, double *w) {
  if (!h || !w) return ST_ERR_USAGE;
  HCHK(h, hipSetDevice(h->device));
  return download_rows(h, h->d_w.p, w);
}
extern "C" int st_get_xb(st_handle h, double *xb) {
  if (!h || !xb) return ST_ERR_USAGE;
  HCHK(h, hipSetDevice(h->device));
  return download_rows(h, h->d_xb.p, xb);
}
extern "C" int st_set_beta(st_handle h, const double *Bcoeff) {
  if (!h || !Bcoeff) return ST_ERR_USAGE;
  invalidate_stats(h);
  HCHK(h, hipSetDevice(h->device));
  h->pin_up_slot ^= 1;
  HCHK(h, hipEventSynchronize(h->ev_up[h->pin_up_slot]));
  double *stg = h->pin_up + (size_t)h->pin_up_slot * h->pin_up_len + QMAX;
  std::memcpy(stg, Bcoeff, (size_t)h->p * h->q * sizeof(double));
  HCHK(h, hipMemcpyAsync(h->d_B.p, stg, (size_t)h->p * h->q * sizeof(double), hipMemcpyHostToDevice, h->stream));
  HCHK(h, hipEventRecord(h->ev_up[h->pin_up_slot], h->stream));
  {
    ProfScope ps(h, 4);
    const int grid = (int)((h->n_all + NT - 1) / NT);
    hipLaunchKernelGGL(k_xb, dim3(grid), dim3(NT), 0, h->stream, h->d_X.p, h->d_mv.p, h->d_B.p, h->n_all, h->p, h->d_xb.p);
  }
  HCHK(h, hipGetLastError());
  return ST_OK;
}
extern "C" int st_set_tausq_inv(st_handle h, const double *t) {
  if (!h || !t) return ST_ERR_USAGE;
  for (int j = 0; j < h->q; ++j) h->tausq_inv[j] = t[j];
  HCHK(h, hipSetDevice(h->device));
  h->pin_up_slot ^= 1;
  HCHK(h, hipEventSynchronize(h->ev_up[h->pin_up_slot]));
  double *stg = h->pin_up + (size_t)h->pin_up_slot * h->pin_up_len;
  std::memcpy(stg, h->tausq_inv, QMAX * sizeof(double));
  HCHK(h, hipMemcpyAsync(h->d_tsq.p, stg, QMAX * sizeof(double), hipMemcpyHostToDevice, h->stream));
  HCHK(h, hipEventRecord(h->ev_up[h->pin_up_slot], h->stream));
  return ST_OK;
}
static int settle_top(st_handle h) {
  if (h->top_pending) { HCHK(h, hipSetDevice(h->device)); HCHK(h, hipStreamWaitEvent(h->stream, h->ev_top, 0)); }
  return ST_OK;
}
static int complete_leaf(st_handle h, int slot) {
  const int phys = h->slot_map[slot];
  if (!h->leaf_pending[phys]) return ST_OK;
  HCHK(h, hipSetDevice(h->device));
  const CovPar &cp = h->leaf_cp[phys];
  ProfScope phase(h, 0, -2, 0);
  for (int g = 0; g < h->n_actual_groups; ++g) {
    const LevelInfo &L = h->levels[g];
    if (L.vl_off < 0) continue;
    QuadArgs F;
    std::memset(&F, 0, sizeof(F));
    F.blks = h->d_blks.p; F.anc_idx = h->d_anc.p; F.grps = h->d_grps.p + L.grp_first;
    F.quads = h->d_quads.p + L.quad_first + L.qown_lo; F.nquad = L.qown_n;
    F.cx = h->d_cx.p; F.cy = h->d_cy.p; F.mv = h->d_mv.p; F.w = h->d_w.p; F.panels = h->d_panels[phys].p;
    F.errflag = h->d_err.p; F.ldS = L.q_ldS;
    F.gdesc = h->d_gdesc.p + (size_t)L.grp_first * h->gd_stride; F.gd_stride = h->gd_stride;
    F.wave_chol = L.maxM <= 27 ? 1 : 0;
    F.mode = QM_TFROMV; F.vscr = h->d_vleaf.p + L.vl_off; F.vtiles = quad_vtiles(L.q_nkx);
    ProfScope ps(h, 0, g, 0);
#define QT(NU_, NKX_, NKT_) hipLaunchKernelGGL((k_factor_quad<NU_, NKX_, NKT_, false, true>), dim3(L.qown_n), dim3(128 * NU_), L.lds_quad, h->stream, F, cp)
    if (L.q_nkx == 32) QT(4, 32, 8); else if (L.q_nkx == 38) QT(4, 38, 10); else if (L.q_nkx == 44) QT(4, 44, 11); else QT(4, 50, 13);
#undef QT
    HCHK(h, hipGetLastError());
  }
  h->leaf_pending[phys] = false;
  return ST_OK;
}
extern "C" int st_swap(st_handle h) {
  if (!h) return ST_ERR_USAGE;
  if (h->top_pending) {
    h->err = "st_swap between st_factor_begin and the st_factor / st_factor_local that picks its result up";
    return ST_ERR_USAGE;
  }
  { const int rc = complete_leaf(h, 1); if (rc) return rc; }
  std::swap(h->slot_map[0], h->slot_map[1]);
  std::swap(h->theta[0], h->theta[1]);
  h->gram_valid = false;
  std::fill(h->s0_valid.begin(), h->s0_valid.end(), 0);
  return ST_OK;
}
extern "C" int st_synchronize(st_handle h) {
  if (!h) return ST_ERR_USAGE;
  HCHK(h, hipSetDevice(h->device));
  HCHK(h, hipStreamSynchronize(h->stream));
  return ST_OK;
}
extern "C" void *st_stream(st_handle h) { return h ? (void *)h->stream : nullptr; }
extern "C" int st_set_stream(st_handle h, void *stream) {
  if (!h) return ST_ERR_USAGE;
  HCHK(h, hipSetDevice(h->device));
  HCHK(h, hipStreamSynchronize(h->stream));
  prof_harvest(h);
  if (h->stream && !h->ext_stream) (void)hipStreamDestroy(h->stream);
  h->stream = (hipStream_t)stream;
  h->ext_stream = true;
  return ST_OK;
}
extern "C" int st_shard_info(st_handle h, int32_t *rank, int32_t *world, int32_t *cut_level, int64_t *owned_blocks, int64_t *owned_rows) {
  if (!h) return ST_ERR_USAGE;
  if (rank) *rank = h->rank;
  if (world) *world = h->world;
  if (cut_level) *cut_level = h->cut;
  long long ob = 0, orow = 0;
  for (size_t i = 0; i < h->blks.size(); ++i) if (h->blk_owner[i] == h->rank) { ++ob; orow += h->blks[i].m; }
  if (owned_blocks) *owned_blocks = ob;
  if (owned_rows) *owned_rows = orow;
  return ST_OK;
}

static int make_covpar(st_handle h, const double *theta, int ntheta, CovPar *cp) {
  const int q = h->q, ncb = q > 2 ? 3 : 1, npars = 3 * q + ncb, k = q * (q - 1) / 2;
  if (ntheta != npars + k) { h->err = "theta has the wrong length"; return ST_ERR_USAGE; }
  std::memset(cp, 0, sizeof(*cp));
  cp->q = q; cp->ncb = ncb;
  for (int j = 0; j < q; ++j) { cp->ai1[j] = theta[j]; cp->ai2[j] = theta[q + j]; cp->phi[j] = theta[2 * q + j]; }
  for (int j = 0; j < ncb; ++j) cp->tmv[j] = theta[3 * q + j];
  int ix = 0;
  for (int j = 0; j < q; ++j)
    for (int i = j + 1; i < q; ++i) { cp->D[i * q + j] = theta[npars + ix]; cp->D[j * q + i] = theta[npars + ix]; ++ix; }
  finish_covpar(cp);
  return ST_OK;
}

template <bool BIG, int MODE>
static void launch_factor(st_handle h, const LevelInfo &L, FactorArgs &A, const CovPar &cp, hipStream_t st = nullptr) {
  int grid = A.nlist;
  if (BIG) {
    grid = std::min(grid, h->scratch_wgs);
    A.scratch = h->d_scratch.p; A.scratch_stride = h->scratch_stride;
  }
  hipLaunchKernelGGL((k_factor<BIG, MODE>), dim3(grid), dim3(NT), L.lds_factor, st ? st : h->stream, A, cp);
}

static int reduce_loglik(st_handle h, int phys, double *loglik) {
  {
    ProfScope ps(h, 3);
    launch_sum2(h->stream, h->d_logdet[phys].p, h->d_loglik[phys].p, (int)h->n_blocks, h->d_scalars.p + 8, h->d_scalars.p);
  }
  HCHK(h, hipGetLastError());
  double s[2];
  HCHK(h, hipMemcpyAsync(s, h->d_scalars.p, 2 * sizeof(double), hipMemcpyDeviceToHost, h->stream));
  HCHK(h, hipStreamSynchronize(h->stream));
  *loglik = s[0] + s[1];
  return ST_OK;
}

static int read_err(st_handle h, int *code) {
  int e[2];
  HCHK(h, hipMemcpyAsync(e, h->d_err.p, 2 * sizeof(int), hipMemcpyDeviceToHost, h->stream));
  HCHK(h, hipStreamSynchronize(h->stream));
  *code = (e[0] == INT_MAX) ? 0 : (e[0] & 15);
  return ST_OK;
}
static int reset_err(st_handle h) {
  const int init[2] = {INT_MAX, 0};
  HCHK(h, hipMemcpyAsync(h->d_err.p, init, 2 * sizeof(int), hipMemcpyHostToDevice, h->stream));
  return ST_OK;
}


static int factor_launch(st_handle h, int phys, const CovPar &cp, int g_lo = 0, int g_hi = INT_MAX, hipStream_t st = nullptr, int *errflag = nullptr,
// ... 46 lines not shown
#define QLAUNCH(NU_, NKX_, NKT_, R_)     \
  do {                                                                                                                         \
    if (L.isref && F.wave_chol) { route(g, R_); hipLaunchKernelGGL((k_factor_quad<NU_, NKX_, NKT_, true, true>), dim3(L.qown_n), dim3(128 * NU_), L.lds_quad, st, F, cp); } \
    else if (L.isref) { route(g, R_ + 1); hipLaunchKernelGGL((k_factor_quad<NU_, NKX_, NKT_, true, false>), dim3(L.qown_n), dim3(128 * NU_), L.lds_quad, st, F, cp); } \
    else {                                                                                                                     \
      if (vonly && L.vl_off >= 0) { F.mode = QM_VONLY; F.vscr = h->d_vleaf.p + L.vl_off; F.vtiles = quad_vtiles(NKX_); *deferred = true; } \
      route(g, R_ + 2); hipLaunchKernelGGL((k_factor_quad<NU_, NKX_, NKT_, false, true>), dim3(L.qown_n), dim3(128 * NU_), L.lds_quad, st, F, cp); } \
  } while (0)
        if (L.q_nkx == 32) QLAUNCH(4, 32, 8, R_QUAD32_REF_WCH); else if (L.q_nkx == 38) QLAUNCH(4, 38, 10, R_QUAD38_REF_WCH);
        else if (L.q_nkx == 44) QLAUNCH(4, 44, 11, R_QUAD44_REF_WCH); else QLAUNCH(4, 50, 13, R_QUAD50_REF_WCH);
#undef QLAUNCH
      } else if (L.fast) {
        FastArgs F;
        std::memset(&F, 0, sizeof(F));
        F.blks = h->d_blks.p; F.anc_idx = h->d_anc.p; F.grps = h->d_grps.p + L.grp_first + L.gown_lo; F.ngrp = L.gown_n;
        F.cx = h->d_cx.p; F.cy = h->d_cy.p; F.mv = h->d_mv.p; F.w = h->d_w.p; F.panels = h->d_panels[phys].p;
        F.logdet_c = h->d_logdet[phys].p; F.loglik_c = h->d_loglik[phys].p; F.errflag = errflag;
        F.Pm4 = L.Pm4; F.ldKV = L.ldKV; F.ldS = L.ldS; F.SRm = L.SRm; F.stage_dbl = L.stage_dbl;
        F.gdesc = h->d_gdesc.p + (size_t)(L.grp_first + L.gown_lo) * h->gd_stride; F.gd_stride = h->gd_stride;
        route(g, R_FACTOR_MFMA);
        hipLaunchKernelGGL(k_factor_mfma, dim3(L.gown_n), dim3(NT), L.lds_fast, st, F, cp);
      } else if (L.bigmfma && h->sw.factor_gen == 3 && L.lchain) {
        LcArgs C;
        std::memset(&C, 0, sizeof(C));
        C.blks = h->d_blks.p; C.anc_idx = h->d_anc.p; C.slabs = h->d_lcslabs.p + L.lc_first; C.nslab = L.lc_count;
        C.cx = h->d_cx.p; C.cy = h->d_cy.p; C.mv = h->d_mv.p; C.w_in = h->d_w.p; C.panels = h->d_panels[phys].p;
        C.rowtmp = h->d_lcrow.p; C.n_rows = h->n_all; C.errflag = errflag;
        C.errcode = L.lchain_ref ? 2 : 3;
        C.vscr = L.lchain_ref ? h->d_vscr.p : nullptr;
        if (L.lchain == 96) { route(g, R_LCHAIN96); hipLaunchKernelGGL((k_factor_lchain<96>), dim3(L.lc_count), dim3(LC_NT), lc_dyn_doubles(96) * 8, st, C, cp); }
        else { route(g, R_LCHAIN136); hipLaunchKernelGGL((k_factor_lchain<136>), dim3(L.lc_count), dim3(LC_NT), lc_dyn_doubles(136) * 8, st, C, cp); }
        if (L.lchain_ref) {
          A.vscr = h->d_vscr.p; A.voff = h->d_rfvoff.p + L.rf_first; A.hvrow = h->d_lcrow.p;
          route(g, R_REF_FINISH);
          hipLaunchKernelGGL(k_factor_ref_finish, dim3(std::min(A.nlist, 2 * h->sm_count)), dim3(BM_NT), L.lds_ref_finish, st, A, cp);
        } else {
          route(g, R_LCHAIN_SCALARS);
          hipLaunchKernelGGL(k_lchain_scalars, dim3((A.nlist + 255) / 256), dim3(256), 0, st, h->d_blks.p, A.list, A.nlist, h->d_lcrow.p, h->n_all,
                             h->d_logdet[phys].p, h->d_loglik[phys].p);
        }
      } else if (L.bigmfma && h->sw.factor_gen == 3 && L.wide_count > 0) {
        WideArgs W;
        std::memset(&W, 0, sizeof(W));
        W.blks = h->d_blks.p; W.anc_idx = h->d_anc.p; W.list = h->d_lvl.p + L.first + L.own_lo; W.groups = h->d_wgrps.p + L.wide_first;
        W.ngroups = L.wide_count; W.cx = h->d_cx.p; W.cy = h->d_cy.p; W.mv = h->d_mv.p; W.w_in = h->d_w.p; W.panels = h->d_panels[phys].p;
        W.logdet_c = h->d_logdet[phys].p; W.loglik_c = h->d_loglik[phys].p; W.errflag = errflag; W.scratch = h->d_scratch.p;
        W.scratch_stride = h->scratch_stride; W.maxP = L.maxP; W.maxN = L.wide_maxN; W.maxM = L.maxM; W.maxMa = L.maxMa; W.ldS = L.bm_ldS;
        route(g, R_FACTOR_WIDE);
        hipLaunchKernelGGL((k_factor_wide<WG_JT>), dim3(std::min(L.wide_count, h->sm_count)), dim3(WG_NT), L.lds_wide, st, W, cp);
      } else if (L.bigmfma && h->sw.factor_gen == 3) {
        A.scratch = h->d_scratch.p; A.scratch_stride = h->scratch_stride; A.SR = L.bm_ldS;
        if (L.maxM <= 48) { route(g, R_BIGMFMA3); hipLaunchKernelGGL((k_factor_bigmfma<3, 5, 34>), dim3(std::min(A.nlist, h->sm_count)), dim3(BM_NT), L.lds_bigmfma, st, A, cp); }
        else if (L.maxM <= 64) { route(g, R_BIGMFMA4); hipLaunchKernelGGL((k_factor_bigmfma<4, 5, 34>), dim3(std::min(A.nlist, h->sm_count)), dim3(BM_NT), L.lds_bigmfma, st, A, cp); }
        else { route(g, R_BIGMFMA5); hipLaunchKernelGGL((k_factor_bigmfma<5, 3, 24>), dim3(std::min(A.nlist, h->sm_count)), dim3(BM_NT), L.lds_bigmfma, st, A, cp); }
      } else if (L.big_factor) { route(g, R_FACTOR_SCRATCH); launch_factor<true, MODE_FACTOR>(h, L, A, cp, st); }
      else { route(g, R_FACTOR_LDS); launch_factor<false, MODE_FACTOR>(h, L, A, cp, st); }
    }
    HCHK(h, hipGetLastError());
  }
  return ST_OK;
}


extern "C" int st_factor_ahead_levels(st_handle h) { return (h && h->async_top && !h->async_top_off) ? h->g_top : 0; }
extern "C" int st_factor_ahead_enable(st_handle h, int enable) {
  if (!h) return ST_ERR_USAGE;
  h->async_top_off = !enable;
  return ST_OK;
}
extern "C" int st_factor_begin(st_handle h, int slot, const double *theta, int ntheta) {
  if (!h || !theta || slot < 0 || slot > 1) return ST_ERR_USAGE;
  if (!h->async_top || h->async_top_off) return ST_OK;
  HCHK(h, hipSetDevice(h->device));
  CovPar cp;
  int rc = make_covpar(h, theta, ntheta, &cp);
  if (rc) return rc;
  if (h->top_pending) HCHK(h, hipStreamWaitEvent(h->stream2, h->ev_top, 0));
  HCHK(h, hipEventRecord(h->ev_main, h->stream));
  HCHK(h, hipStreamWaitEvent(h->stream2, h->ev_main, 0));
  const int init[2] = {INT_MAX, 0};
  HCHK(h, hipMemcpyAsync(h->d_err2.p, init, 2 * sizeof(int), hipMemcpyHostToDevice, h->stream2));
  const int phys = h->slot_map[slot];
  h->leaf_pending[phys] = false;
  h->prof_suspend = true;
  rc = factor_launch(h, phys, cp, 0, h->g_top, h->stream2, h->d_err2.p);
  h->prof_suspend = false;
  if (rc) return rc;
  HCHK(h, hipEventRecord(h->ev_top, h->stream2));
  h->top_pending = true; h->top_phys = phys; h->top_theta.assign(theta, theta + ntheta);
  return ST_OK;
}
static int fix_top_comps(st_handle h, int phys);
static int run_stats(st_handle h, hipStream_t st);
static int stats_begin(st_handle h) {
  if (!h->stream2 || h->stats_valid) return ST_OK;
  HCHK(h, hipEventRecord(h->ev_main, h->stream));
  HCHK(h, hipStreamWaitEvent(h->stream2, h->ev_main, 0));
  int rc = run_stats(h, h->stream2);
  if (rc) return rc;
  const size_t nq = (size_t)h->p * h->q + h->q;
  h->stats_prefetched = nq <= 40;
  if (h->stats_prefetched) HCHK(h, hipMemcpyAsync(h->pin + 20, h->d_stats.p, nq * sizeof(double), hipMemcpyDeviceToHost, h->stream2));
  HCHK(h, hipEventRecord(h->ev_stats, h->stream2));
  h->stats_on_stream2 = true;
  return ST_OK;
}

static int factor_local(st_handle h, int slot, const double *theta, int ntheta, bool vonly);
extern "C" int st_factor_local(st_handle h, int slot, const double *theta, int ntheta) { return factor_local(h, slot, theta, ntheta, false); }
static int factor_local(st_handle h, int slot, const double *theta, int ntheta, bool vonly) {
  if (!h || !theta || slot < 0 || slot > 1) return ST_ERR_USAGE;
  HCHK(h, hipSetDevice(h->device));
  CovPar cp;
  int rc = make_covpar(h, theta, ntheta, &cp);
  if (rc) return rc;
  h->theta[slot].assign(theta, theta + ntheta);
  if (slot == 0) { h->gram_valid = false; std::fill(h->s0_valid.begin(), h->s0_valid.end(), 0); }
  rc = reset_err(h);
  if (rc) return rc;
  const int phys = h->slot_map[slot];
  h->leaf_pending[phys] = false;
  if (slot == 1) { rc = stats_begin(h); if (rc) return rc; }
  bool reuse = false;
  if (h->top_pending) {
    HCHK(h, hipStreamWaitEvent(h->stream, h->ev_top, 0));
    reuse = h->top_phys == phys && (int)h->top_theta.size() == ntheta && std::equal(theta, theta + ntheta, h->top_theta.begin());
    h->top_pending = false;
  }
  bool deferred = false;
  rc = factor_launch(h, phys, cp, reuse ? h->g_top : 0, INT_MAX, nullptr, nullptr, vonly, &deferred);
  if (deferred) { h->leaf_pending[phys] = true; h->leaf_cp[phys] = cp; }
  if (rc || !reuse) return rc;
  rc = fix_top_comps(h, phys);
  if (rc) return rc;
  hipLaunchKernelGGL(k_merge_err, dim3(1), dim3(64), 0, h->stream, h->d_err.p, h->d_err2.p);
  HCHK(h, hipGetLastError());
  return ST_OK;
}

extern "C" int st_mg_pack_comps(st_handle h, int slot, void **dev_ptr, int64_t *len) {
  if (!h || slot < 0 || slot > 1) return ST_ERR_USAGE;
  HCHK(h, hipSetDevice(h->device));
  { const int rc0 = settle_top(h); if (rc0) return rc0; }
  const int phys = h->slot_map[slot], nb = (int)h->n_blocks;
  {
    ProfScope ps(h, 3);
    hipLaunchKernelGGL(k_pack_comps, dim3((std::max(nb, h->world) + NT - 1) / NT), dim3(NT), 0, h->stream, h->d_logdet[phys].p,
                       h->d_loglik[phys].p, h->d_blkmask.p, nb, h->d_err.p, h->rank, h->world, h->d_comm.p);
  }
  HCHK(h, hipGetLastError());
  if (dev_ptr) *dev_ptr = h->d_comm.p;
  if (len) *len = 2 * (int64_t)nb + h->world;
  return ST_OK;
}

extern "C" int st_mg_finish(st_handle h, double *loglik) {
  if (!h) return ST_ERR_USAGE;
  HCHK(h, hipSetDevice(h->device));
  const int nb = (int)h->n_blocks;
  {
    ProfScope ps(h, 3);
    launch_sum2(h->stream, h->d_comm.p, h->d_comm.p + nb, nb, h->d_scalars.p + 8, h->d_scalars.p);
  }
  HCHK(h, hipGetLastError());
  double s2[2], errw[64];
  HCHK(h, hipMemcpyAsync(s2, h->d_scalars.p, 2 * sizeof(double), hipMemcpyDeviceToHost, h->stream));
  HCHK(h, hipMemcpyAsync(errw, h->d_comm.p + 2 * (size_t)nb, h->world * sizeof(double), hipMemcpyDeviceToHost, h->stream));
  HCHK(h, hipStreamSynchronize(h->stream));
  int best = INT_MAX;
  for (int r = 0; r < h->world; ++r) if (errw[r] > 0.5) best = std::min(best, (int)errw[r]);
  if (best != INT_MAX) return best & 15;
  if (loglik) *loglik = s2[0] + s2[1];
  return ST_OK;
}

#define NCHK(h, call)                                                                                        \
  do {                                                                                                        \
    ncclResult_t r_ = (call);                                                                                 \
    if (r_ != ncclSuccess) { (h)->err = std::string(#call) + ": " + ncclGetErrorString(r_); return ST_ERR_HIP; } \
  } while (0)

static int exchange_comps_and_finish(st_handle h, int slot, double *loglik) {
  void *ptr = nullptr;
  int64_t len = 0;
  int rc = st_mg_pack_comps(h, slot, &ptr, &len);
  if (rc) return rc;
  {
    ProfScope ps(h, 7);
    NCHK(h, ncclAllReduce(ptr, ptr, (size_t)len, ncclDouble, ncclSum, h->comm, h->stream));
  }
  return st_mg_finish(h, loglik);
}

extern "C" int st_comm_unique_id(void *out, int32_t cap) {
  if (!out || cap < (int32_t)sizeof(ncclUniqueId)) return ST_ERR_USAGE;
  ncclUniqueId id;
  if (ncclGetUniqueId(&id) != ncclSuccess) return ST_ERR_HIP;
  std::memcpy(out, &id, sizeof(id));
  return (int)sizeof(id);
}
extern "C" int st_comm_init(st_handle h, const void *unique_id) {
  if (!h || !unique_id) return ST_ERR_USAGE;
  HCHK(h, hipSetDevice(h->device));
  ncclUniqueId id;
// ... 13 lines not shown
  }
  int rc = factor_enqueue(h, slot, theta, ntheta, false);
  if (rc) return rc;
  return st_factor_finish(h, loglik);
}
extern "C" int st_factor_is_async(st_handle h) { return (h && !(h->world > 1 || h->comm)) ? 1 : 0; }
extern "C" int st_factor_enqueue(st_handle h, int slot, const double *theta, int ntheta) {
  return factor_enqueue(h, slot, theta, ntheta, h && h->defer_leaf && slot == 1);
}
static int factor_enqueue(st_handle h, int slot, const double *theta, int ntheta, bool vonly) {
  if (!h || !theta || slot < 0 || slot > 1) return ST_ERR_USAGE;
  if (h->factor_open) { h->err = "st_factor_enqueue: the previous one has not been finished"; return ST_ERR_USAGE; }
  if (h->world > 1 || h->comm) {
    h->factor_open = true; h->factor_open_slot = slot; h->top_theta_open.assign(theta, theta + ntheta);
    return ST_OK;
  }
  int rc = factor_local(h, slot, theta, ntheta, vonly);
  if (rc) return rc;
  {
    ProfScope ps(h, 3);
    const int phys = h->slot_map[slot];
    launch_sum2(h->stream, h->d_logdet[phys].p, h->d_loglik[phys].p, (int)h->n_blocks, h->d_scalars.p + 8, h->d_scalars.p);
  }
  HCHK(h, hipGetLastError());
  HCHK(h, hipMemcpyAsync(h->pin + 12, h->d_scalars.p, 2 * sizeof(double), hipMemcpyDeviceToHost, h->stream));
  HCHK(h, hipMemcpyAsync(h->pin + 14, h->d_err.p, 2 * sizeof(int), hipMemcpyDeviceToHost, h->stream));
  HCHK(h, hipEventRecord(h->ev_factor, h->stream));
  h->factor_open = true; h->factor_open_slot = slot; h->top_theta_open.clear();
  return ST_OK;
}
extern "C" int st_factor_finish(st_handle h, double *loglik) {
  if (!h) return ST_ERR_USAGE;
  if (!h->factor_open) { h->err = "st_factor_finish without st_factor_enqueue"; return ST_ERR_USAGE; }
  h->factor_open = false;
  if (h->world > 1 || h->comm) {
    if (!h->comm) { h->err = "world > 1: call st_comm_init first, or use st_factor_local / st_mg_pack_comps / (all-reduce) / st_mg_finish"; return ST_ERR_USAGE; }
    int rc = st_factor_local(h, h->factor_open_slot, h->top_theta_open.data(), (int)h->top_theta_open.size());
    if (rc) return rc;
    return exchange_comps_and_finish(h, h->factor_open_slot, loglik);
  }
  HCHK(h, hipSetDevice(h->device));
  HCHK(h, hipEventSynchronize(h->ev_factor));
  const int e0 = ((const int *)(h->pin + 14))[0];
  if (e0 != INT_MAX) return e0 & 15;
  if (loglik) *loglik = h->pin[12] + h->pin[13];
  return ST_OK;
}

static int gather_w_scatter(st_handle h);
extern "C" int st_sample_w_loglik(st_handle h, const double *z, uint64_t seed, uint32_t iter, int slot, double *loglik) {
  if (!h || slot < 0 || slot > 1) return ST_ERR_USAGE;
  { const int rc0 = complete_leaf(h, slot); if (rc0) return rc0; }
  if (h->world > 1 || h->comm) {
    if (!h->comm) {
      int rc = st_sample_w(h, z, seed, iter);
      if (rc) return rc;
      return st_loglik_w(h, slot, loglik);
    }
    int rc = st_sample_w_local(h, z, seed, iter);
    if (rc) return rc;
    if (h->top_len > 0) {
      ProfScope ps(h, 7);
      NCHK(h, ncclAllReduce(h->d_acc.p + h->top_off, h->d_acc.p + h->top_off, (size_t)h->top_len, ncclDouble, ncclSum, h->comm, h->stream));
    }
    rc = st_sample_w_top(h);
    if (rc) return rc;
    void *pw = nullptr, *pr = nullptr, *pc = nullptr;
    int64_t lw = 0, lc = 0;
    rc = st_mg_gather_w_pack(h, &pw, &pr, &lw);
    if (rc) return rc;
    rc = st_loglik_local(h, slot);
    if (rc) return rc;
    rc = st_mg_pack_comps(h, slot, &pc, &lc);
    if (rc) return rc;
    {
      ProfScope ps(h, 7);
      NCHK(h, ncclGroupStart());
      NCHK(h, ncclAllGather(pw, pr, (size_t)lw, ncclDouble, h->comm, h->stream));
      NCHK(h, ncclAllReduce(pc, pc, (size_t)lc, ncclDouble, ncclSum, h->comm, h->stream));
      NCHK(h, ncclGroupEnd());
    }
    rc = gather_w_scatter(h);
    if (rc) return rc;
    invalidate_stats(h);
    const int nb = (int)h->n_blocks;
    {
      ProfScope ps(h, 3);
      launch_sum2(h->stream, h->d_comm.p, h->d_comm.p + nb, nb, h->d_scalars.p + 8, h->d_scalars.p);
    }
    HCHK(h, hipGetLastError());
    double s2[2], errw[64], errc[64];
    HCHK(h, hipMemcpyAsync(errw, h->d_gerr.p, h->world * sizeof(double), hipMemcpyDeviceToHost, h->stream));
    HCHK(h, hipMemcpyAsync(s2, h->d_scalars.p, 2 * sizeof(double), hipMemcpyDeviceToHost, h->stream));
    HCHK(h, hipMemcpyAsync(errc, h->d_comm.p + 2 * (size_t)nb, h->world * sizeof(double), hipMemcpyDeviceToHost, h->stream));
    HCHK(h, hipStreamSynchronize(h->stream));
    int best = INT_MAX;
    for (int r = 0; r < h->world; ++r) if (errw[r] > 0.5) best = std::min(best, (int)errw[r]);
    if (best != INT_MAX) return best & 15;
    for (int r = 0; r < h->world; ++r) if (errc[r] > 0.5) best = std::min(best, (int)errc[r]);
    if (best != INT_MAX) return best & 15;
    if (loglik) *loglik = s2[0] + s2[1];
    return ST_OK;
  }
  int rc = st_sample_w_local(h, z, seed, iter);
  if (rc) return rc;
  rc = st_sample_w_top(h);
  if (rc) return rc;
  HCHK(h, hipMemcpyAsync(h->pin + 2, h->d_err.p, 2 * sizeof(int), hipMemcpyDeviceToHost, h->stream));
  rc = st_loglik_local(h, slot);
  if (rc) return rc;
  {
    ProfScope ps(h, 3);
    const int phys = h->slot_map[slot];
    launch_sum2(h->stream, h->d_logdet[phys].p, h->d_loglik[phys].p, (int)h->n_blocks, h->d_scalars.p + 8, h->d_scalars.p);
  }
  HCHK(h, hipGetLastError());
  HCHK(h, hipMemcpyAsync(h->pin, h->d_scalars.p, 2 * sizeof(double), hipMemcpyDeviceToHost, h->stream));
  HCHK(h, hipStreamSynchronize(h->stream));
  const int e0 = ((const int *)(h->pin + 2))[0];
  if (e0 != INT_MAX) return e0 & 15;
  if (loglik) *loglik = h->pin[0] + h->pin[1];
  return ST_OK;
}

extern "C" int st_sample_w_loglik_begin(st_handle h, const double *z, uint64_t seed, uint32_t iter, int slot) {
  if (!h || slot < 0 || slot > 1) return ST_ERR_USAGE;
  if (h->c_pending) return ST_ERR_USAGE;
  { const int rc0 = complete_leaf(h, slot); if (rc0) return rc0; }
  if (h->world > 1 || h->comm) {
    h->c_ll = 0.0;
    h->c_rc = st_sample_w_loglik(h, z, seed, iter, slot, &h->c_ll);
    if (h->c_rc < 0) return h->c_rc;
    h->c_pending = true;
    return ST_OK;
  }
  int rc = st_sample_w_local(h, z, seed, iter);
  if (rc) return rc;
  rc = st_sample_w_top(h);
  if (rc) return rc;
  HCHK(h, hipMemcpyAsync(h->pin + 10, h->d_err.p, 2 * sizeof(int), hipMemcpyDeviceToHost, h->stream));
  rc = st_loglik_local(h, slot);
  if (rc) return rc;
  {
    ProfScope ps(h, 3);
    const int phys = h->slot_map[slot];
    launch_sum2(h->stream, h->d_logdet[phys].p, h->d_loglik[phys].p, (int)h->n_blocks, h->d_scalars.p + 8, h->d_scalars.p);
  }
  HCHK(h, hipGetLastError());
  HCHK(h, hipMemcpyAsync(h->pin + 8, h->d_scalars.p, 2 * sizeof(double), hipMemcpyDeviceToHost, h->stream));
  h->c_rc = INT_MIN;
  h->c_pending = true;
  return ST_OK;
}
extern "C" int st_sample_w_loglik_end(st_handle h, double *loglik) {
  if (!h || !h->c_pending) return ST_ERR_USAGE;
  h->c_pending = false;
  if (h->c_rc != INT_MIN) {
    if (h->c_rc == ST_OK && loglik) *loglik = h->c_ll;
    return h->c_rc;
  }
  HCHK(h, hipStreamSynchronize(h->stream));
  const int e0 = ((const int *)(h->pin + 10))[0];
  if (e0 != INT_MAX) return e0 & 15;
  if (loglik) *loglik = h->pin[8] + h->pin[9];
  return ST_OK;
}

static int gen_or_upload_z(st_handle h, const double *z, uint64_t seed, uint32_t iter, unsigned stream_id, double *dst) {
  if (z) return upload_rows(h, z, dst);
  {
    ProfScope ps(h, 5);
    const int grid = (int)((h->n_all + NT - 1) / NT);
    hipLaunchKernelGGL(k_normals, dim3(grid), dim3(NT), 0, h->stream, dst, h->d_dev2model.p, h->n_all, iter, stream_id,
                       (unsigned long long)seed);
  }
  HCHK(h, hipGetLastError());
  return ST_OK;
}

static int sample_launch(st_handle h, int g_hi, int g_lo) {
  const int phys = h->slot_map[0];
  for (int g = g_hi - 1; g >= g_lo; --g) {
    const LevelInfo &L = h->levels[g];
    int *route = h->route_b.data() + 2 * (size_t)g;
    route[0] = route[1] = R_NONE;
    if ((L.fast ? L.gown_n : L.own_n) == 0) continue;
    SampleArgs A;
    std::memset(&A, 0, sizeof(A));
    A.blks = h->d_blks.p; A.anc_idx = h->d_anc.p; A.dch_idx = h->d_dch.p; A.list = h->d_lvl.p + L.first + L.own_lo; A.nlist = L.own_n;
    A.panels = h->d_panels[phys].p; A.w = h->d_w.p; A.y = h->d_y.p; A.xb = h->d_xb.p; A.z = h->d_z.p; A.mv = h->d_mv.p;
    A.obs = h->d_obs.p; A.acc = h->d_acc.p; A.errflag = h->d_err.p; A.maxP = L.maxP; A.maxM = L.maxM; A.maxLd = L.maxLd;
    for (int j = 0; j < QMAX; ++j) A.tausq_inv[j] = h->tausq_inv[j];
    A.do_gram = (h->gram_valid && h->cache_gram) ? 0 : 1;
    A.no_fwd = h->limited ? 1 : 0;
    A.lds_sq = (L.big_sample && L.sample_sq) ? 2 : 0;
    A.s0 = h->d_s0.p; A.s0off = h->d_s0off.p;
    {
      ProfScope ps(h, 1, h->n_actual_groups + g);
      if (L.fast) {
        SampleFastArgs F;
        std::memset(&F, 0, sizeof(F));
        F.do_gram = A.do_gram; F.no_fwd = A.no_fwd;
        F.blks = h->d_blks.p; F.anc_idx = h->d_anc.p; F.dch_idx = h->d_dch.p; F.grps = h->d_grps.p + L.grp_first + L.gown_lo; F.ngrp = L.gown_n;
        F.panels = h->d_panels[phys].p; F.w = h->d_w.p; F.y = h->d_y.p; F.xb = h->d_xb.p; F.z = h->d_z.p; F.mv = h->d_mv.p;
        F.acc = h->d_acc.p; F.errflag = h->d_err.p; F.ldN = L.ldN; F.Mr4 = L.Mr4; F.Mrows = L.Mrows; F.maxP = L.maxP; F.av_dbl = L.av_dbl;
        F.gdesc = h->d_gdesc.p + (size_t)(L.grp_first + L.gown_lo) * h->gd_stride; F.gd_stride = h->gd_stride;
        for (int j = 0; j < QMAX; ++j) F.tausq_inv[j] = h->tausq_inv[j];
        const bool lean_ok = h->sw.sample_lean && !(!L.isref && L.maxP > 255);
        F.gdesc_all = h->d_gdesc.p;
        auto splits = [&](int gq) {
          const LevelInfo &Lq = h->levels[gq];
          const bool lean_q = h->sw.sample_lean && !(!Lq.isref && Lq.maxP > 255);
          return Lq.fast && lean_q && h->sw.split_gram && (h->sw.split_gram == 2 || (Lq.isref && Lq.gown_n >= 32 * h->sm_count));
        };
        const bool direct_parent = F.do_gram && h->gram_direct_level == g && splits(g) && h->levels[g + 1].gown_n > 0;
        if (F.do_gram && lean_ok && g == h->gram_direct_level + 1 && h->gram_direct_level >= 0 && splits(g - 1) && h->levels[g - 1].gown_n > 0) F.do_gram = 0;
        if (F.do_gram && lean_ok && h->sw.split_gram && (h->sw.split_gram == 2 || (L.isref && L.gown_n >= 32 * h->sm_count))) {
          if (direct_parent) { route[0] = R_GRAM_DIRECT; hipLaunchKernelGGL(k_gram_direct, dim3(L.gown_n), dim3(NT), 0, h->stream, F); }
          else { route[0] = R_GRAM; hipLaunchKernelGGL(k_gram, dim3(L.gown_n), dim3(NT), 0, h->stream, F); }
          F.do_gram = 0;
        }
        if (!(F.do_gram || !lean_ok) && L.isref) {
          F.s0 = h->d_s0.p; F.s0off = h->d_s0off.p;
          F.s0_mode = !h->cache_gram ? 0 : (h->s0_valid[g] ? 2 : 1);
          if (h->cache_gram) h->s0_valid[g] = 1;
        }
        if (F.do_gram || !lean_ok) { route[1] = R_SAMPLE_MFMA; hipLaunchKernelGGL(k_sample_mfma, dim3(L.gown_n), dim3(NT), L.lds_sfast, h->stream, F); }
        else if (!L.isref) {
          const int need = (L.maxJ + 1) / 2;
          if (h->sw.leaf_seg && need <= 4 && L.maxMa <= 32) { route[1] = R_LEAF_SEG4; hipLaunchKernelGGL((k_sample_leaf_seg<4>), dim3(L.gown_n), dim3(NT), ((size_t)4 * 64 * 4 + 3 * 32) * 8, h->stream, F); }
          else if (h->sw.leaf_seg && need <= 6 && L.maxMa <= 32) { route[1] = R_LEAF_SEG6; hipLaunchKernelGGL((k_sample_leaf_seg<6>), dim3(L.gown_n), dim3(NT), ((size_t)4 * 64 * 6 + 3 * 32) * 8, h->stream, F); }
          else { route[1] = R_SAMPLE_LEAF; hipLaunchKernelGGL(k_sample_leaf, dim3(L.gown_n), dim3(NT), ((size_t)L.maxP + 32 + 4 * 256 + 3 * 32) * 8, h->stream, F); }
        }
        else if (h->sw.sample_wave && L.maxM <= 27 && (h->sw.sample_wave == 2 || L.gown_n >= 8 * h->sm_count)) {
          const size_t per = (((size_t)h->gd_stride + L.maxP + 32 + L.av_dbl + 64 + (size_t)std::max(L.maxM, 1) * CH_LD + 1) & ~(size_t)1);
          F.ldN = (int)per; F.Mrows = L.maxM;
          route[1] = R_SAMPLE_WAVE;
          hipLaunchKernelGGL(k_sample_wave, dim3((L.gown_n + NT / 64 - 1) / (NT / 64)), dim3(NT), per * 8 * (NT / 64), h->stream, F);
        } else {
          F.av_dbl = L.av_dbl + 224;
          if (h->sw.sample_lat && L.gown_n <= 2 * h->sm_count) { route[1] = R_SAMPLE_LEAN_LAT; hipLaunchKernelGGL((k_sample_lean<true>), dim3(L.gown_n), dim3(NT), L.lds_slean, h->stream, F); }
          else { route[1] = R_SAMPLE_LEAN; hipLaunchKernelGGL((k_sample_lean<false>), dim3(L.gown_n), dim3(NT), L.lds_slean, h->stream, F); }
        }
      } else {
        if (A.do_gram && L.big_sample && h->sw.gram_big) {
          GramBigArgs Gb;
          std::memset(&Gb, 0, sizeof(Gb));
          Gb.blks = h->d_blks.p; Gb.anc_idx = h->d_anc.p; Gb.dch_idx = h->d_dch.p; Gb.list = A.list; Gb.nlist = A.nlist;
          Gb.panels = A.panels; Gb.acc = A.acc; Gb.s0 = A.s0; Gb.s0off = A.s0off; Gb.no_fwd = A.no_fwd;
          bool all_big = true;
          for (const auto &L2 : h->levels) all_big = all_big && (L2.count == 0 || L2.big_sample);
          Gb.mirror = all_big ? 0 : 1;
          route[0] = R_GRAM_BIG;
          hipLaunchKernelGGL(k_gram_big, dim3(A.nlist), dim3(NT), 0, h->stream, Gb);
          A.do_gram = 0;
        }
        if (L.big_sample) {
          A.scratch = h->d_scratch.p; A.scratch_stride = h->scratch_stride;
          if (L.isref) { route[1] = R_SAMPLE_BIG_REF; hipLaunchKernelGGL((k_sample<true, false>), dim3(std::min(L.own_n, h->scratch_wgs)), dim3(NT), L.lds_sample, h->stream, A); }
          else if (h->sw.leaf_wide && !A.do_gram && L.maxM <= 64 && L.maxMa <= 96 && L.maxJ <= 8) {
            route[1] = R_SAMPLE_LEAF_WIDE;
            hipLaunchKernelGGL(k_sample_leaf_wide, dim3(std::min(L.own_n, 16 * h->sm_count)), dim3(NT), ((size_t)4 * 64 * 12 + 3 * 64) * 8, h->stream, A);
          } else { route[1] = R_SAMPLE_BIG_LEAF; hipLaunchKernelGGL((k_sample<true, true>), dim3(std::min(L.own_n, h->scratch_wgs)), dim3(NT), L.lds_sample, h->stream, A); }
        } else {
          route[1] = R_SAMPLE_SMALL;
          hipLaunchKernelGGL((k_sample<false>), dim3(L.own_n), dim3(NT), L.lds_sample, h->stream, A);
        }
      }
    }
    HCHK(h, hipGetLastError());
  }
  return ST_OK;
}

extern "C" int st_sample_w_local(st_handle h, const double *z, uint64_t seed, uint32_t iter) {
  if (!h) return ST_ERR_USAGE;
  invalidate_stats(h);
  HCHK(h, hipSetDevice(h->device));
  int rc = gen_or_upload_z(h, z, seed, iter, 0u, h->d_z.p);
  if (rc) return rc;
  h->z_valid = true;
  rc = reset_err(h);
  if (rc) return rc;
  rc = sample_launch(h, h->n_actual_groups, std::min(h->cut, h->n_actual_groups));
  if (rc) return rc;
  for (auto &zr : h->top_zero) HCHK(h, hipMemsetAsync(h->d_acc.p + zr.first, 0, (size_t)zr.second * sizeof(double), h->stream));
  return ST_OK;
}
extern "C" int st_mg_top_region(st_handle h, void **dev_ptr, int64_t *len) {
  if (!h) return ST_ERR_USAGE;
  if (dev_ptr) *dev_ptr = h->d_acc.p + h->top_off;
  if (len) *len = h->top_len;
  return ST_OK;
}
extern "C" int st_sample_w_top(st_handle h) {
  if (!h) return ST_ERR_USAGE;
  invalidate_stats(h);
  HCHK(h, hipSetDevice(h->device));
  const int rc = sample_launch(h, std::min(h->cut, h->n_actual_groups), 0);
  if (rc == ST_OK) h->gram_valid = true;
  return rc;
}
extern "C" int st_mg_pack_w(st_handle h, void **dev_ptr, int64_t *len) {
  if (!h) return ST_ERR_USAGE;
  HCHK(h, hipSetDevice(h->device));
  const long long nn = std::max<long long>(h->n_all, h->world);
  hipLaunchKernelGGL(k_pack_w, dim3((unsigned)((nn + NT - 1) / NT)), dim3(NT), 0, h->stream, h->d_w.p, h->d_rowmask.p, h->n_all, h->d_err.p,
                     h->rank, h->world, h->d_tmp_n.p);
  HCHK(h, hipGetLastError());
  if (dev_ptr) *dev_ptr = h->d_tmp_n.p;
  if (len) *len = h->n_all + h->world;
  return ST_OK;
}
extern "C" int st_mg_unpack_w(st_handle h) {
  if (!h) return ST_ERR_USAGE;
  invalidate_stats(h);
  HCHK(h, hipSetDevice(h->device));
  double errw[64];
  HCHK(h, hipMemcpyAsync(h->d_w.p, h->d_tmp_n.p, (size_t)h->n_all * sizeof(double), hipMemcpyDeviceToDevice, h->stream));
  HCHK(h, hipMemcpyAsync(errw, h->d_tmp_n.p + h->n_all, h->world * sizeof(double), hipMemcpyDeviceToHost, h->stream));
  HCHK(h, hipStreamSynchronize(h->stream));
  int best = INT_MAX;
  for (int r = 0; r < h->world; ++r) if (errw[r] > 0.5) best = std::min(best, (int)errw[r]);
  return best == INT_MAX ? ST_OK : (best & 15);
}

extern "C" int st_mg_gather_w_pack(st_handle h, void **send_ptr, void **recv_ptr, int64_t *count_per_rank) {
  if (!h) return ST_ERR_USAGE;
  HCHK(h, hipSetDevice(h->device));
  const int cnt = h->gather_cnt;
  double *mine = h->d_gather.p + (size_t)h->rank * cnt;
  hipLaunchKernelGGL(k_gather_pack, dim3((cnt + NT - 1) / NT), dim3(NT), 0, h->stream, h->d_w.p, h->d_gidx.p + (size_t)h->rank * cnt, cnt,
                     h->d_err.p, mine);
  HCHK(h, hipGetLastError());
  if (send_ptr) *send_ptr = mine;
  if (recv_ptr) *recv_ptr = h->d_gather.p;
  if (count_per_rank) *count_per_rank = cnt;
  return ST_OK;
}
static int gather_w_scatter(st_handle h) {
  const long long total = (long long)h->world * h->gather_cnt;
  hipLaunchKernelGGL(k_gather_unpack, dim3((unsigned)((total + NT - 1) / NT)), dim3(NT), 0, h->stream, h->d_gather.p, h->d_gidx.p, h->gather_cnt,
                     total, h->d_w.p, h->d_gerr.p);
  HCHK(h, hipGetLastError());
  return ST_OK;
}
extern "C" int st_mg_gather_w_unpack(st_handle h) {
  if (!h) return ST_ERR_USAGE;
  invalidate_stats(h);
  HCHK(h, hipSetDevice(h->device));
  int rc = gather_w_scatter(h);
  if (rc) return rc;
  double errw[64];
  HCHK(h, hipMemcpyAsync(errw, h->d_gerr.p, h->world * sizeof(double), hipMemcpyDeviceToHost, h->stream));
  HCHK(h, hipStreamSynchronize(h->stream));
  int best = INT_MAX;
  for (int r = 0; r < h->world; ++r) if (errw[r] > 0.5) best = std::min(best, (int)errw[r]);
  return best == INT_MAX ? ST_OK : (best & 15);
}

extern "C" int st_sample_w(st_handle h, const double *z, uint64_t seed, uint32_t iter) {
  if (!h) return ST_ERR_USAGE;
  if (h->world > 1 || h->comm) {
    if (!h->comm) { h->err = "world > 1: call st_comm_init first, or use st_sample_w_local / st_mg_top_region / st_sample_w_top / st_mg_pack_w / st_mg_unpack_w"; return ST_ERR_USAGE; }
    int rc = st_sample_w_local(h, z, seed, iter);
    if (rc) return rc;
    if (h->top_len > 0) {
      ProfScope ps(h, 7);
      NCHK(h, ncclAllReduce(h->d_acc.p + h->top_off, h->d_acc.p + h->top_off, (size_t)h->top_len, ncclDouble, ncclSum, h->comm, h->stream));
    }
    rc = st_sample_w_top(h);
    if (rc) return rc;
    void *snd = nullptr, *rcv = nullptr;
    int64_t cnt = 0;
    rc = st_mg_gather_w_pack(h, &snd, &rcv, &cnt);
    if (rc) return rc;
    {
      ProfScope ps(h, 7);
      NCHK(h, ncclAllGather(snd, rcv, (size_t)cnt, ncclDouble, h->comm, h->stream));
    }
    return st_mg_gather_w_unpack(h);
  }
  int rc = st_sample_w_local(h, z, seed, iter);
  if (rc) return rc;
  rc = st_sample_w_top(h);
  if (rc) return rc;
  int code = 0;
  rc = read_err(h, &code);
  if (rc) return rc;
  return code;
}

extern "C" int st_loglik_local(st_handle h, int slot) {
  if (!h || slot < 0 || slot > 1) return ST_ERR_USAGE;
  HCHK(h, hipSetDevice(h->device));
  if (slot == 1) { const int rc0 = settle_top(h); if (rc0) return rc0; }
  { const int rc0 = complete_leaf(h, slot); if (rc0) return rc0; }
  const int phys = h->slot_map[slot];
  int maxP = 0, maxM = 0;
  for (auto &L : h->levels) { maxP = std::max(maxP, L.maxP); maxM = std::max(maxM, L.maxM); }
  const size_t lds = lds_loglik_bytes(maxP, maxM);
  LoglikArgs A;
  A.blks = h->d_blks.p; A.anc_idx = h->d_anc.p; A.list = h->d_ownslow.p; A.nlist = (int)h->own_obs_slow.size();
  A.panels = h->d_panels[phys].p; A.w = h->d_w.p; A.loglik_c = h->d_loglik[phys].p; A.maxP = maxP; A.maxM = maxM;
  {
    ProfScope ps(h, 2);
    if (A.nlist > 0) hipLaunchKernelGGL(k_loglik, dim3(A.nlist), dim3(NT), lds, h->stream, A);
    if (!h->own_grp_list.empty()) {
      LoglikGrpArgs Gr;
      Gr.blks = h->d_blks.p; Gr.anc_idx = h->d_anc.p; Gr.grps = h->d_grps.p; Gr.list = h->d_owngrp.p; Gr.nlist = (int)h->own_grp_list.size();
      Gr.panels = h->d_panels[phys].p; Gr.w = h->d_w.p; Gr.loglik_c = h->d_loglik[phys].p; Gr.maxP = maxP;
      Gr.gdesc = h->d_gdesc.p; Gr.gd_stride = h->gd_stride;
      hipLaunchKernelGGL(k_loglik_grp, dim3(Gr.nlist), dim3(NT), (size_t)(maxP + 32) * sizeof(double), h->stream, Gr);
    }
  }
  HCHK(h, hipGetLastError());
  HCHK(h, reset_err(h) == ST_OK ? hipSuccess : hipErrorUnknown);
  return ST_OK;
}
static int fix_top_comps(st_handle h, int phys) {
  if (h->n_toplist == 0) return ST_OK;
  int maxP = 0, maxM = 0;
  for (int g = 0; g < h->g_top; ++g) { maxP = std::max(maxP, h->levels[g].maxP); maxM = std::max(maxM, h->levels[g].maxM); }
  LoglikArgs A;
  A.blks = h->d_blks.p; A.anc_idx = h->d_anc.p; A.list = h->d_toplist.p; A.nlist = h->n_toplist;
  A.panels = h->d_panels[phys].p; A.w = h->d_w.p; A.loglik_c = h->d_loglik[phys].p; A.maxP = maxP; A.maxM = maxM;
  {
    ProfScope ps(h, 0, h->g_top > 0 ? h->g_top - 1 : 0);
    hipLaunchKernelGGL(k_loglik, dim3(A.nlist), dim3(NT), lds_loglik_bytes(maxP, maxM), h->stream, A);
  }
  HCHK(h, hipGetLastError());
  return ST_OK;
}
extern "C" int st_loglik_w(st_handle h, int slot, double *loglik) {
  if (!h) return ST_ERR_USAGE;
  if (slot >= 0 && slot <= 1) { const int rc0 = complete_leaf(h, slot); if (rc0) return rc0; }
  if (h->world > 1 || h->comm) {
    if (!h->comm) { h->err = "world > 1: call st_comm_init first, or use st_loglik_local / st_mg_pack_comps / (all-reduce) / st_mg_finish"; return ST_ERR_USAGE; }
    int rc = st_loglik_local(h, slot);
    if (rc) return rc;
    return exchange_comps_and_finish(h, slot, loglik);
  }
  int rc = st_loglik_local(h, slot);
  if (rc) return rc;
  double ll = 0.0;
  rc = reduce_loglik(h, h->slot_map[slot], &ll);
  if (rc) return rc;
  if (loglik) *loglik = ll;
  return ST_OK;
}

extern "C" int st_predict(st_handle h, int theta_changed) {
  (void)theta_changed;
  if (!h) return ST_ERR_USAGE;
  if (h->pred_list.empty()) return ST_OK;
  invalidate_stats(h);
  if (!h->z_valid) { h->err = "st_predict needs the normals of a preceding st_sample_w (spamtree_model.cpp:1325)"; return ST_ERR_USAGE; }
  if (h->theta[0].empty()) { h->err = "st_predict before st_factor(slot 0)"; return ST_ERR_USAGE; }
  HCHK(h, hipSetDevice(h->device));
  CovPar cp;
  int rc = make_covpar(h, h->theta[0].data(), (int)h->theta[0].size(), &cp);
  if (rc) return rc;
  const LevelInfo &L = h->pred_info;
  if (h->pred_nkx > 0 && h->pred_quad_count > 0) {
    QuadArgs F;
    std::memset(&F, 0, sizeof(F));
    F.blks = h->d_blks.p; F.anc_idx = h->d_anc.p; F.grps = h->d_grps.p + h->pred_grp_first;
    F.quads = h->d_quads.p + h->pred_quad_first; F.nquad = h->pred_quad_count;
    F.cx = h->d_cx.p; F.cy = h->d_cy.p; F.mv = h->d_mv.p; F.w = h->d_w.p; F.panels = h->d_panels[h->slot_map[0]].p;
    F.logdet_c = nullptr; F.loglik_c = nullptr; F.errflag = h->d_err.p; F.ldS = quad_lds_stride(h->pred_nkx);
    F.gdesc = h->d_gdesc.p + (size_t)h->pred_grp_first * h->gd_stride; F.gd_stride = h->gd_stride;
    F.wave_chol = 1; F.predict = 1; F.z = h->d_z.p; F.w_out = h->d_w.p;
    {
      ProfScope ps(h, 6);
      const dim3 grid(h->pred_quad_count), blk(128 * 4);
      if (h->pred_nkx == 32) { h->route_p = R_QUAD32_LEAF; hipLaunchKernelGGL((k_factor_quad<4, 32, 8, false, true>), grid, blk, h->pred_lds, h->stream, F, cp); }
      else if (h->pred_nkx == 38) { h->route_p = R_QUAD38_LEAF; hipLaunchKernelGGL((k_factor_quad<4, 38, 10, false, true>), grid, blk, h->pred_lds, h->stream, F, cp); }
      else if (h->pred_nkx == 44) { h->route_p = R_QUAD44_LEAF; hipLaunchKernelGGL((k_factor_quad<4, 44, 11, false, true>), grid, blk, h->pred_lds, h->stream, F, cp); }
      else { h->route_p = R_QUAD50_LEAF; hipLaunchKernelGGL((k_factor_quad<4, 50, 13, false, true>), grid, blk, h->pred_lds, h->stream, F, cp); }
    }
    HCHK(h, hipGetLastError());
    HCHK(h, hipStreamSynchronize(h->stream));
    return ST_OK;
  }
  FactorArgs A;
  std::memset(&A, 0, sizeof(A));
  A.blks = h->d_blks.p; A.anc_idx = h->d_anc.p; A.list = h->d_pred.p; A.nlist = (int)h->pred_list.size();
  A.cx = h->d_cx.p; A.cy = h->d_cy.p; A.mv = h->d_mv.p; A.w_in = h->d_w.p; A.w_out = h->d_w.p; A.z = h->d_z.p;
  A.panels = h->d_panels[h->slot_map[0]].p; A.logdet_c = nullptr; A.loglik_c = nullptr; A.errflag = h->d_err.p;
  A.maxP = L.maxP; A.maxM = L.maxM; A.maxMa = L.maxMa; A.SR = L.big_factor ? 4 : 8;
  {
    ProfScope ps(h, 6);
    if (L.big_factor) { h->route_p = R_PREDICT_SCRATCH; launch_factor<true, MODE_PREDICT>(h, L, A, cp); }
    else { h->route_p = R_PREDICT_LDS; launch_factor<false, MODE_PREDICT>(h, L, A, cp); }
  }
  HCHK(h, hipGetLastError());
  HCHK(h, hipStreamSynchronize(h->stream));
  return ST_OK;
}

static int run_stats(st_handle h, hipStream_t st = nullptr) {
  const int nq = h->p * h->q + h->q;
  if (h->stats_valid) return ST_OK;
  if (!st) st = h->stream;
  {
    ProfScope ps(h, 4, -1, 1, st);
    hipLaunchKernelGGL(k_stats, dim3(STATS_WG), dim3(NT), 0, st, h->d_X.p, h->d_y.p, h->d_w.p, h->d_xb.p, h->d_mv.p, h->d_obs.p,
                       h->d_partner.p, h->n_all, h->p, h->q, h->d_partial.p);
    hipLaunchKernelGGL(k_stats_final, dim3(nq), dim3(NT), 0, st, h->d_partial.p, STATS_WG, nq, h->d_stats.p);
  }
  HCHK(h, hipGetLastError());
  h->stats_valid = true;
  return ST_OK;
}
static int fetch_stats(st_handle h) {
  if (h->stats_valid && h->host_stats_valid) return ST_OK;
  int rc = run_stats(h);
  if (rc) return rc;
  const size_t nq = (size_t)h->p * h->q + h->q;
  h->host_stats.resize(nq);
  if (h->stats_on_stream2) {
    if (h->stats_prefetched) {
      HCHK(h, hipEventSynchronize(h->ev_stats));
      HCHK(h, hipStreamWaitEvent(h->stream, h->ev_stats, 0));
      h->stats_on_stream2 = false;
      for (size_t i = 0; i < nq; ++i) h->host_stats[i] = h->pin[20 + i];
      h->host_stats_valid = true;
      return ST_OK;
    }
    HCHK(h, hipStreamWaitEvent(h->stream, h->ev_stats, 0));
    h->stats_on_stream2 = false;
  }
  HCHK(h, hipMemcpyAsync(h->host_stats.data(), h->d_stats.p, nq * sizeof(double), hipMemcpyDeviceToHost, h->stream));
  HCHK(h, hipStreamSynchronize(h->stream));
  h->host_stats_valid = true;
  return ST_OK;
}
extern "C" int st_beta_stats(st_handle h, double *xty) {
  if (!h || !xty) return ST_ERR_USAGE;
// ... 712 lines not shown
```

spamtree_amd/csrc/st_device.hpp:

```cpp
#pragma once
#include <hip/hip_runtime.h>

#include <algorithm>
#include <climits>
#include <cmath>
#include <cstdint>
#include <cstdio>
#include <cstdlib>
#include <cstring>
#include <numeric>
#include <string>
#include <vector>

#include "spamtree_hip.h"
#include <rccl/rccl.h>

#define NT 256
#define MAXJ ST_MAX_ANCESTORS
#define QMAX ST_MAX_Q
#define HL2PI (-0.91893853320467274178032973640562)

struct CovPar {
  int q;
  int ncb;
// ... 572 lines not shown
    __syncthreads();
    double w = 0.0;
    if (rowok && ib == kb) {
      for (int c = i; c < k1; ++c) w += S[(size_t)c * lds_ + i] * vec[c];
    }
    __syncthreads();
    if (rowok && ib == kb) { vec[i] = w; t = w; }
    __syncthreads();
    if (rowok && ib < kb) {
      for (int c = k0; c < k1; ++c) t -= S[(size_t)c * lds_ + i] * vec[c];
    }
  }
  if (rowok) bv[i] = t;
  __syncthreads();
}

#ifdef FM_STAMPS
static __device__ unsigned long long g_stamps[16];
#define STAMP_DECL unsigned long long st_acc[16] = {0,0,0,0,0,0,0,0,0,0,0,0,0,0,0,0}; unsigned long long st_t0 = clock64(), st_t1 = 0;
#define STAMP(slot) do { st_t1 = clock64(); st_acc[slot] += st_t1 - st_t0; st_t0 = st_t1; } while (0)
static __device__ int g_stamp_level = -1;
#define STAMP_FLUSH_IF(c_) do { if (threadIdx.x == 0 && (c_)) { for (int q_ = 0; q_ < 16; ++q_) atomicAdd(&g_stamps[q_], st_acc[q_]); } } while (0)
#define STAMP_FLUSH STAMP_FLUSH_IF(g_stamp_level < 0)
#define STAMP_FLUSH_LEVEL(l_) STAMP_FLUSH_IF(g_stamp_level < 0 || g_stamp_level == (l_))
#ifdef ST_STAMP_SUFFIX
#define ST_STAMP_CAT2(a, b) a##b
#define ST_STAMP_CAT(a, b) ST_STAMP_CAT2(a, b)
extern "C" int ST_STAMP_CAT(st_debug_stamp_level, ST_STAMP_SUFFIX)(int level) { (void)hipMemcpyToSymbol(HIP_SYMBOL(g_stamp_level), &level, sizeof(int)); return 0; }
extern "C" int ST_STAMP_CAT(st_debug_stamps, ST_STAMP_SUFFIX)(unsigned long long *out, int reset) {
  if (out) (void)hipMemcpyFromSymbol(out, HIP_SYMBOL(g_stamps), sizeof(unsigned long long) * 16);
  if (reset) { unsigned long long z[16] = {0}; (void)hipMemcpyToSymbol(HIP_SYMBOL(g_stamps), z, sizeof(z)); }
  return 0;
}
#endif
#else
#define STAMP_DECL
#define STAMP(slot) do {} while (0)
#define STAMP_FLUSH do {} while (0)
#define STAMP_FLUSH_LEVEL(l_) do {} while (0)
#endif


struct Grp {
  long long row0;
  int blk0, nblk;
  int M, P;
};

#define GD_MAXW 272
struct GdHead {
  long long row0, acc_off;
  int M, P, nanc, nblk, isref, level, ndch, acc_len, blk0;
};
__device__ __forceinline__ GdHead gd_unpack(const long long *s_gd, int tid, int *s_am, int *s_ao, long long *s_arow, long long *s_apan,
                                            long long *s_aoff, long long *s_bpan, long long *s_brow, int *s_bld, long long *s_coff) {
  GdHead H;
  auto sll = [](long long v) {
    const int lo = __builtin_amdgcn_readfirstlane((int)(v & 0xffffffffLL)), hi = __builtin_amdgcn_readfirstlane((int)(v >> 32));
    return ((long long)hi << 32) | (unsigned int)lo;
  };
  auto slo = [](long long v) { return __builtin_amdgcn_readfirstlane((int)(v & 0xffffffffLL)); };
  auto shi = [](long long v) { return __builtin_amdgcn_readfirstlane((int)(v >> 32)); };
  H.row0 = sll(s_gd[0]); H.acc_off = sll(s_gd[1]);
  H.M = slo(s_gd[2]); H.P = shi(s_gd[2]);
  H.nanc = slo(s_gd[3]); H.nblk = shi(s_gd[3]);
  H.isref = slo(s_gd[4]); H.level = shi(s_gd[4]);
  H.ndch = slo(s_gd[5]); H.acc_len = shi(s_gd[5]);
  H.blk0 = slo(s_gd[6]);
  if (tid < H.nanc) {
    const long long *a = s_gd + 8 + 4 * tid;
    s_am[tid] = (int)(a[0] & 0xffffffffLL); s_ao[tid] = (int)(a[0] >> 32);
    s_arow[tid] = a[1];
    if (s_apan) s_apan[tid] = a[2];
    if (s_aoff) s_aoff[tid] = a[3];
  }
  if (tid == 0) { s_ao[H.nanc] = H.P; if (s_aoff) s_aoff[H.nanc] = s_gd[7]; }
  if (tid >= 64 && tid < 64 + H.nblk) {
    const long long *b = s_gd + 8 + 4 * H.nanc + 3 * (tid - 64);
    s_bpan[tid - 64] = b[0]; s_brow[tid - 64] = b[1]; s_bld[tid - 64] = (int)b[2];
  }
  if (s_coff && tid >= 128 && tid < 128 + H.ndch) s_coff[tid - 128] = s_gd[8 + 4 * H.nanc + 3 * H.nblk + (tid - 128)];
  return H;
}
```

Measured before the change: 241.1.

## Hand off per-ancestor segment dot products from loglik kernel to sampler

```diff
diff --git a/include/spamtree_hip.h b/include/spamtree_hip.h
--- a/include/spamtree_hip.h
+++ b/include/spamtree_hip.h
@@ -77,6 +77,7 @@
 int st_sample_w(st_handle h, const double *z, uint64_t seed, uint32_t iter);
 
 int st_loglik_w(st_handle h, int slot, double *loglik);
+int st_seg_handoff_counts(st_handle h, int64_t *stored, int64_t *used);
 
 int st_sample_w_loglik(st_handle h, const double *z, uint64_t seed, uint32_t iter, int slot, double *loglik);
 int st_sample_w_loglik_begin(st_handle h, const double *z, uint64_t seed, uint32_t iter, int slot);
diff --git a/spamtree_amd/_lib.py b/spamtree_amd/_lib.py
--- a/spamtree_amd/_lib.py
+++ b/spamtree_amd/_lib.py
@@ -37,6 +37,7 @@
     "st_swap": (C.c_int, [H]),
     "st_sample_w": (C.c_int, [H, c_dp, C.c_uint64, C.c_uint32]),
     "st_loglik_w": (C.c_int, [H, C.c_int, c_dp]),
+    "st_seg_handoff_counts": (C.c_int, [H, c_ip, c_ip]),
     "st_sample_w_loglik": (C.c_int, [H, c_dp, C.c_uint64, C.c_uint32, C.c_int, c_dp]),
     "st_sample_w_loglik_begin": (C.c_int, [H, c_dp, C.c_uint64, C.c_uint32, C.c_int]),
     "st_sample_w_loglik_end": (C.c_int, [H, c_dp]),
diff --git a/spamtree_amd/csrc/misc_kernels.hpp b/spamtree_amd/csrc/misc_kernels.hpp
--- a/spamtree_amd/csrc/misc_kernels.hpp
+++ b/spamtree_amd/csrc/misc_kernels.hpp
@@ -24,8 +24,12 @@
   int maxP;
   const long long *gdesc;
   int gd_stride;
+  double *segc;
+  const long long *segoff;
+  int seg_ps;
 };
 
+#define LOGLIK_SEG_RS 2
 #define SUM2_WG 64
 #define STATS_WG 1024
 struct QtArgs {
@@ -106,8 +110,11 @@
   __shared__ long long s_gd[GD_MAXW];
   const int tid = threadIdx.x, lane = tid & 63, wid = tid >> 6;
   double *wv = lds;
+  long long sgo = -1;
   {
-    const long long *gd = A.gdesc + (size_t)A.list[blockIdx.x] * A.gd_stride;
+    const int g = A.list[blockIdx.x];
+    const long long *gd = A.gdesc + (size_t)g * A.gd_stride;
+    if (A.segc) sgo = A.segoff[g];
     for (int i = tid; i < A.gd_stride; i += NT) s_gd[i] = gd[i];
   }
   __syncthreads();
@@ -158,6 +165,26 @@
       }
       acc = wave_sum(acc);
       if (lane == 0 && j < 32) s_e2[j] = acc * acc;
+      if (sgo >= 0) {
+        constexpr int RS = LOGLIK_SEG_RS;
+        const int q = rr & (RS - 1);
+        int tl = tid;
+        asm volatile("" : "+v"(tl));
+        const int ln = tl & 63;
+        double *stg = wv + A.maxP + 32 + (size_t)((tl >> 6) * RS) * A.seg_ps;
+#pragma unroll
+        for (int c = 0; c < 5; ++c) {
+          const int k = ln + 64 * c;
+          if (k < P) stg[q * A.seg_ps + k] = v[rr][c];
+        }
+        if (q == RS - 1) {
+          asm volatile("s_waitcnt lgkmcnt(0)" ::: "memory");
+          if (ln < RS * J) {
+            const int qq = ln / J, t = ln - qq * J, jr = j - 4 * (RS - 1 - qq);
+            if (jr < M) A.segc[sgo + (size_t)jr * J + t] = seg_walk(stg + qq * A.seg_ps + s_ao[t], wv + s_ao[t], s_am[t]);
+          }
+        }
+      }
     }
   }
   __syncthreads();
diff --git a/spamtree_amd/csrc/sample_kernels.hpp b/spamtree_amd/csrc/sample_kernels.hpp
--- a/spamtree_amd/csrc/sample_kernels.hpp
+++ b/spamtree_amd/csrc/sample_kernels.hpp
@@ -59,6 +59,9 @@
   double *s0;
   const long long *s0off;
   int s0_mode;
+  const double *segc;
+  const long long *segoff;
+  int seg_mode;
 };
 #define GRAM_DIRECT_MAXCH 4
 
@@ -1026,12 +1029,14 @@
     const int per = A.ngrp >> 3;
     if (gidx < per * 8) gidx = (gidx & 7) * per + (gidx >> 3);
   }
+  const long long sgo = A.seg_mode ? A.segoff[gidx] : -1;
   for (int i = tid; i < A.gd_stride; i += NT) s_gd[i] = A.gdesc[(size_t)gidx * A.gd_stride + i];
   __syncthreads();
   const GdHead B0 = gd_unpack(s_gd, tid, s_am, s_ao, s_arow, nullptr, s_aoff, s_bpan, s_brow, s_bld, s_coff);
   const Grp G = {B0.row0, B0.blk0, B0.nblk, B0.M, B0.P};
   const int M = G.M, P = G.P, J = B0.nanc;
   const bool refgrp = B0.isref != 0;
+  const bool seg_load = refgrp && sgo >= 0;
   if (tid == 0) { s_fail = 0; s_nch = B0.ndch; }
   const long long so = (refgrp && A.s0off && A.s0_mode) ? A.s0off[B0.blk0] : -1;
   const bool s0_load = so >= 0 && A.s0_mode == 2;
@@ -1059,7 +1064,7 @@
     lds_barrier();
     double wreg = 0.0;
     int wk = -1;
-    if (tid < P) {
+    if (tid < P && !seg_load) {
       int t = 0;
       while (t + 1 < J && tid >= s_ao[t + 1]) ++t;
       wk = tid; wreg = A.w[s_arow[t] + (tid - s_ao[t])];
@@ -1076,7 +1081,8 @@
       const int ma = J ? s_am[t] : 0;
       const double *row = A.panels + s_rowoff[r] + (J ? s_ao[t] : 0);
 #pragma unroll
-      for (int jj = 0; jj < 28; ++jj) xq[jj] = (idx < mj && jj < ma) ? row[jj] : 0.0;
+      for (int jj = 0; jj < 28; ++jj) xq[jj] = (idx < mj && jj < ma && !seg_load) ? row[jj] : 0.0;
+      if (seg_load) xq[0] = (idx < mj) ? A.segc[sgo + idx] : 0.0;
     }
 #pragma unroll
     for (int cc = 0; cc < 4; ++cc)
@@ -1098,7 +1104,7 @@
     if (rowthr) t_ = A.tausq_inv[mv_];
     if (tid >= 32 && tid < 64) { const int j = tid - 32; tsq[j] = t_; yx[j] = y_ - xb_; zc[j] = z_; rjv[j] = r_; }
     if (wk >= 0) wv[wk] = wreg;
-    for (int k = NT + tid; k < P; k += NT) {
+    for (int k = NT + tid; k < P && !seg_load; k += NT) {
       int t = 0;
       while (t + 1 < J && k >= s_ao[t + 1]) ++t;
       wv[k] = A.w[s_arow[t] + (k - s_ao[t])];
@@ -1132,7 +1138,7 @@
     tsq[j] = t_; yx[j] = y_; zc[j] = z_; rjv[j] = r_; s_cb[j] = bi; s_rowoff[j] = ro;
   }
   __syncthreads();
-  for (int k = tid; k < P; k += NT) {
+  for (int k = tid; k < P && !seg_load; k += NT) {
     int t = 0;
     while (t + 1 < J && k >= s_ao[t + 1]) ++t;
     wv[k] = A.w[s_arow[t] + (k - s_ao[t])];
@@ -1145,6 +1151,12 @@
   }
   __syncthreads();
   }
+  if (seg_load) {
+    for (int idx = tid; idx < M * J; idx += NT) {
+      const int r = idx / J, t = idx - r * J;
+      seg[t * 32 + r] = (LAT && idx == tid) ? xq[0] : A.segc[sgo + idx];
+    }
+  } else
   for (int idx = tid; idx < M * J; idx += NT) {
     const int r = idx / J, t = idx - r * J;
     const int ma = s_am[t], oa = s_ao[t];
@@ -1153,14 +1165,14 @@
     double a = 0.0;
     if (LAT && idx == tid && ma <= 28) {
 #pragma unroll
-      for (int jj = 0; jj < 28; ++jj) a += xq[jj] * ((jj < ma) ? wa[jj] : 0.0);
+      for (int jj = 0; jj < 28; ++jj) a = seg_step(a, xq[jj], (jj < ma) ? wa[jj] : 0.0);
     } else
     for (int j0 = 0; j0 < ma; j0 += 16) {
       double x[16];
 #pragma unroll
       for (int jj = 0; jj < 16; ++jj) x[jj] = (j0 + jj < ma) ? row[j0 + jj] : 0.0;
 #pragma unroll
-      for (int jj = 0; jj < 16; ++jj) a += x[jj] * ((j0 + jj < ma) ? wa[j0 + jj] : 0.0);
+      for (int jj = 0; jj < 16; ++jj) a = seg_step(a, x[jj], (j0 + jj < ma) ? wa[j0 + jj] : 0.0);
     }
     seg[t * 32 + r] = a;
   }
@@ -1306,6 +1318,7 @@
   double *tv = seg + A.av_dbl, *ev = tv + 32;
   double *Rc = ev + 32;
   if (lane == 0) s_failw[wid] = 0;
+  const long long sgo = A.seg_mode ? A.segoff[gidx] : -1;
   for (int i = lane; i < A.gd_stride; i += 64) s_gd[i] = A.gdesc[(size_t)gidx * A.gd_stride + i];
   WSYNC();
   auto slo = [](long long v) { return __builtin_amdgcn_readfirstlane((int)(v & 0xffffffffLL)); };
@@ -1324,14 +1337,32 @@
   const int li = min(lane, 31);
   double tsq = 0.0, yx = 0.0, zc = 0.0;
   if (row) { const long long r = row0 + lane; tsq = A.tausq_inv[A.mv[r]]; yx = A.y[r] - A.xb[r]; zc = A.z[r]; }
-  for (int k = lane; k < P; k += 64) {
+  for (int k = lane; k < P && sgo < 0; k += 64) {
     int t = 0;
     for (int j = 1; j < J; ++j) t += k >= ao_of(j) ? 1 : 0;
     wv[k] = A.w[s_gd[8 + 4 * t + 1] + (k - ao_of(t))];
   }
   const int PS = P | 1;
   const int RG = min(4, (A.Mrows * CH_LD) / PS);
-  if (RG >= 1) {
+  if (sgo >= 0) {
+    double sreg[4];
+#pragma unroll
+    for (int q = 0; q < 4; ++q) sreg[q] = (lane + 64 * q < M * J) ? A.segc[sgo + lane + 64 * q] : 0.0;
+    for (int idx = lane; idx < M * M; idx += 64) {
+      const int i = idx / M, j = idx - i * M;
+      Rc[i * CH_LD + j] = (j <= i) ? A.panels[bpan + (size_t)i * bld + P + j] : 0.0;
+    }
+#pragma unroll
+    for (int q = 0; q < 4; ++q) {
+      const int idx = lane + 64 * q, r = idx / max(J, 1), t = idx - r * J;
+      if (idx < M * J) seg[t * 32 + r] = sreg[q];
+    }
+    for (int idx = lane + 256; idx < M * J; idx += 64) {
+      const int r = idx / J, t = idx - r * J;
+      seg[t * 32 + r] = A.segc[sgo + idx];
+    }
+    WSYNC();
+  } else if (RG >= 1) {
     constexpr int NRI = (27 * 27 + 63) / 64;
     double rireg[NRI];
 #pragma unroll
@@ -1365,9 +1396,7 @@
           const int ma = am_of(t), oa = ao_of(t);
           const double *srow = stg + rr * PS + oa;
           const double *wa = wv + oa;
-          double a = 0.0;
-          for (int j = 0; j < ma; ++j) a += srow[j] * wa[j];
-          seg[t * 32 + r] = a;
+          seg[t * 32 + r] = seg_walk(srow, wa, ma);
         }
       }
     }
@@ -1395,7 +1424,7 @@
 #pragma unroll
       for (int jj = 0; jj < 16; ++jj) x[jj] = (j0 + jj < ma) ? prow[j0 + jj] : 0.0;
 #pragma unroll
-      for (int jj = 0; jj < 16; ++jj) a += x[jj] * ((j0 + jj < ma) ? wa[j0 + jj] : 0.0);
+      for (int jj = 0; jj < 16; ++jj) a = seg_step(a, x[jj], (j0 + jj < ma) ? wa[j0 + jj] : 0.0);
     }
     seg[t * 32 + r] = a;
   }
diff --git a/spamtree_amd/csrc/spamtree_hip.hip b/spamtree_amd/csrc/spamtree_hip.hip
--- a/spamtree_amd/csrc/spamtree_hip.hip
+++ b/spamtree_amd/csrc/spamtree_hip.hip
@@ -92,7 +92,7 @@
 struct Switches {
   int wide = 1, split_gram = 1, sample_wave = 1;
   bool lchain = true, lchain_ref = true, gram_big = true, gram_direct = true, sample_lean = true, sample_lat = true,
-       leaf_seg = true, leaf_wide = true, async_top = true;
+       leaf_seg = true, leaf_wide = true, async_top = true, seg_handoff = true;
   int lchain_ref_min = 1;
   int factor_gen = 3;
   int quad_units = 0;
@@ -109,6 +109,7 @@
   s.lchain = level("SPAMTREE_LCHAIN"); s.lchain_ref = level("SPAMTREE_LCHAIN_REF"); s.gram_big = level("SPAMTREE_GRAM_BIG");
   s.gram_direct = level("SPAMTREE_GRAM_DIRECT"); s.sample_lean = level("SPAMTREE_SAMPLE_LEAN"); s.sample_lat = level("SPAMTREE_SAMPLE_LAT");
   s.leaf_seg = level("SPAMTREE_LEAF_SEG"); s.leaf_wide = level("SPAMTREE_LEAF_WIDE"); s.async_top = level("SPAMTREE_ASYNC_TOP");
+  s.seg_handoff = level("SPAMTREE_SEG_HANDOFF");
   const char *e;
   if ((e = getenv("SPAMTREE_LCHAIN_REF_MIN"))) s.lchain_ref_min = atoi(e);
   if ((e = getenv("SPAMTREE_FACTOR_KERNEL")) && e[0] == '1') s.factor_gen = 1;
@@ -148,6 +149,15 @@
   DevBuf<double> d_lcrow;
   DevBuf<double> d_s0;
   DevBuf<long long> d_s0off;
+  DevBuf<double> d_seg;
+  DevBuf<long long> d_segoff;
+  bool seg_on = false;
+  std::vector<char> seg_level;
+  int seg_levels = 0, seg_ps = 1;
+  int seg_phys = -1;
+  bool seg_valid = false;
+  bool seg_sweep = false;
+  long long seg_stored = 0, seg_used = 0;
   bool c_pending = false;
   int c_rc = 0; double c_ll = 0.0;
   std::vector<long long> gdesc;
@@ -306,6 +316,13 @@
   }
   h->stats_valid = false; h->host_stats_valid = false;
 }
+static void invalidate_w(st_handle_s *h) {
+  invalidate_stats(h);
+  h->seg_valid = false; h->seg_sweep = false;
+}
+static void invalidate_seg_arena(st_handle_s *h, int phys) {
+  if (h->seg_phys == phys) { h->seg_valid = false; h->seg_sweep = false; }
+}
 
 static size_t lds_factor_bytes(int maxP, int maxM, int maxMa, int SR, bool big) {
   size_t dbl = (size_t)3 * (maxP + maxM) + 3 * (size_t)maxM + (size_t)SR * maxP;
@@ -335,7 +352,7 @@
   for (int s = 0; s < 2; ++s) { h->d_logdet[s].free(); h->d_loglik[s].free(); }
   h->d_scalars.free(); h->d_partial.free(); h->d_stats.free(); h->d_scratch.free(); h->d_tmp_n.free(); h->d_tsq.free();
   h->d_mv.free(); h->d_anc.free(); h->d_dch.free(); h->d_lvl.free(); h->d_pred.free(); h->d_allobs.free(); h->d_err.free();
-  h->d_twin.free(); h->d_wgrps.free(); h->d_lcslabs.free(); h->d_lcrow.free(); h->d_rfvoff.free(); h->d_vscr.free(); h->d_vleaf.free(); h->d_s0.free(); h->d_s0off.free(); h->d_obs.free(); h->d_dev2model.free(); h->d_partner.free(); h->d_blks.free(); h->d_grps.free(); h->d_quads.free(); h->d_gdesc.free();
+  h->d_twin.free(); h->d_wgrps.free(); h->d_lcslabs.free(); h->d_lcrow.free(); h->d_rfvoff.free(); h->d_vscr.free(); h->d_vleaf.free(); h->d_s0.free(); h->d_s0off.free(); h->d_seg.free(); h->d_segoff.free(); h->d_obs.free(); h->d_dev2model.free(); h->d_partner.free(); h->d_blks.free(); h->d_grps.free(); h->d_quads.free(); h->d_gdesc.free();
   h->d_ownobs.free(); h->d_owngrp.free(); h->d_ownslow.free(); h->d_rowmask.free(); h->d_blkmask.free(); h->d_comm.free(); h->d_gather.free(); h->d_gidx.free(); h->d_gerr.free(); h->d_err2.free(); h->d_toplist.free();
   if (h->ev_top) (void)hipEventDestroy(h->ev_top);
   if (h->ev_main) (void)hipEventDestroy(h->ev_main);
@@ -1112,6 +1129,31 @@
   }
   for (int b : h->own_obs_list) if (!h->levels[h->blks[b].level].fast) h->own_obs_slow.push_back(b);
   { std::vector<int> a = h->own_grp_list; if (a.empty()) a.push_back(0); CCHK(h->d_owngrp.upload(a)); }
+  h->seg_on = h->sw.seg_handoff && h->world == 1 && !h->force_generic && h->cache_gram && h->sw.sample_lean;
+  if (h->seg_on) {
+    std::vector<long long> segoff(std::max(h->grps.size(), (size_t)1), -1);
+    size_t tot = 0;
+    int maxPref = 0, maxJref = 0;
+    h->seg_level.assign((size_t)std::max(n_actual, 1), 0);
+    for (int g = 0; g < n_actual; ++g) {
+      const LevelInfo &L = h->levels[g];
+      if (!L.fast || !L.isref) continue;
+      bool any = false;
+      for (int k = 0; k < L.grp_count; ++k) {
+        const Grp &G = h->grps[L.grp_first + k];
+        const int J = h->blks[G.blk0].nanc;
+        if (G.nblk != 1 || J == 0) continue;
+        segoff[L.grp_first + k] = (long long)tot;
+        tot += (size_t)G.M * J;
+        maxPref = std::max(maxPref, G.P); maxJref = std::max(maxJref, J);
+        any = true;
+      }
+      h->seg_level[g] = any; h->seg_levels += any ? 1 : 0;
+    }
+    h->seg_ps = maxPref | 1;
+    if (tot == 0 || LOGLIK_SEG_RS * maxJref > 64) h->seg_on = false;
+    else { CCHK(h->d_segoff.upload(segoff)); CCHK(h->d_seg.alloc(tot)); }
+  }
   { std::vector<int> a = h->own_obs_slow; if (a.empty()) a.push_back(0); CCHK(h->d_ownslow.upload(a)); }
   CCHK(h->d_rowmask.upload(rowmask)); CCHK(h->d_blkmask.upload(blkmask));
   CCHK(h->d_comm.alloc((size_t)2 * nb + 64));
@@ -1283,7 +1325,7 @@
 
 extern "C" int st_set_w(st_handle h, const double *w) {
   if (!h || !w) return ST_ERR_USAGE;
-  invalidate_stats(h);
+  invalidate_w(h);
   HCHK(h, hipSetDevice(h->device));
   return upload_rows(h, w, h->d_w.p);
 }
@@ -1335,6 +1377,7 @@
   const int phys = h->slot_map[slot];
   if (!h->leaf_pending[phys]) return ST_OK;
   HCHK(h, hipSetDevice(h->device));
+  invalidate_seg_arena(h, phys);
   const CovPar &cp = h->leaf_cp[phys];
   ProfScope phase(h, 0, -2, 0);
   for (int g = 0; g < h->n_actual_groups; ++g) {
@@ -1369,6 +1412,7 @@
   std::swap(h->theta[0], h->theta[1]);
   h->gram_valid = false;
   std::fill(h->s0_valid.begin(), h->s0_valid.end(), 0);
+  h->seg_valid = false; h->seg_sweep = false;
   return ST_OK;
 }
 extern "C" int st_synchronize(st_handle h) {
@@ -1581,6 +1625,7 @@
   HCHK(h, hipMemcpyAsync(h->d_err2.p, init, 2 * sizeof(int), hipMemcpyHostToDevice, h->stream2));
   const int phys = h->slot_map[slot];
   h->leaf_pending[phys] = false;
+  invalidate_seg_arena(h, phys);
   h->prof_suspend = true;
   rc = factor_launch(h, phys, cp, 0, h->g_top, h->stream2, h->d_err2.p);
   h->prof_suspend = false;
@@ -1614,11 +1659,12 @@
   int rc = make_covpar(h, theta, ntheta, &cp);
   if (rc) return rc;
   h->theta[slot].assign(theta, theta + ntheta);
-  if (slot == 0) { h->gram_valid = false; std::fill(h->s0_valid.begin(), h->s0_valid.end(), 0); }
+  if (slot == 0) { h->gram_valid = false; std::fill(h->s0_valid.begin(), h->s0_valid.end(), 0); h->seg_valid = false; h->seg_sweep = false; }
   rc = reset_err(h);
   if (rc) return rc;
   const int phys = h->slot_map[slot];
   h->leaf_pending[phys] = false;
+  invalidate_seg_arena(h, phys);
   if (slot == 1) { rc = stats_begin(h); if (rc) return rc; }
   bool reuse = false;
   if (h->top_pending) {
@@ -1798,7 +1844,7 @@
     }
     rc = gather_w_scatter(h);
     if (rc) return rc;
-    invalidate_stats(h);
+    invalidate_w(h);
     const int nb = (int)h->n_blocks;
     {
       ProfScope ps(h, 3);
@@ -1924,6 +1970,11 @@
         for (int j = 0; j < QMAX; ++j) F.tausq_inv[j] = h->tausq_inv[j];
         const bool lean_ok = h->sw.sample_lean && !(!L.isref && L.maxP > 255);
         F.gdesc_all = h->d_gdesc.p;
+        auto seg_consume = [&](SampleFastArgs &Fa) {
+          if (!h->seg_sweep || !h->seg_level[g]) return;
+          Fa.segc = h->d_seg.p; Fa.segoff = h->d_segoff.p + L.grp_first + L.gown_lo; Fa.seg_mode = 1;
+          ++h->seg_used;
+        };
         auto splits = [&](int gq) {
           const LevelInfo &Lq = h->levels[gq];
           const bool lean_q = h->sw.sample_lean && !(!Lq.isref && Lq.maxP > 255);
@@ -1951,10 +2002,12 @@
         else if (h->sw.sample_wave && L.maxM <= 27 && (h->sw.sample_wave == 2 || L.gown_n >= 8 * h->sm_count)) {
           const size_t per = (((size_t)h->gd_stride + L.maxP + 32 + L.av_dbl + 64 + (size_t)std::max(L.maxM, 1) * CH_LD + 1) & ~(size_t)1);
           F.ldN = (int)per; F.Mrows = L.maxM;
+          seg_consume(F);
           route[1] = R_SAMPLE_WAVE;
           hipLaunchKernelGGL(k_sample_wave, dim3((L.gown_n + NT / 64 - 1) / (NT / 64)), dim3(NT), per * 8 * (NT / 64), h->stream, F);
         } else {
           F.av_dbl = L.av_dbl + 224;
+          seg_consume(F);
           if (h->sw.sample_lat && L.gown_n <= 2 * h->sm_count) { route[1] = R_SAMPLE_LEAN_LAT; hipLaunchKernelGGL((k_sample_lean<true>), dim3(L.gown_n), dim3(NT), L.lds_slean, h->stream, F); }
           else { route[1] = R_SAMPLE_LEAN; hipLaunchKernelGGL((k_sample_lean<false>), dim3(L.gown_n), dim3(NT), L.lds_slean, h->stream, F); }
         }
@@ -1991,7 +2044,11 @@
 
 extern "C" int st_sample_w_local(st_handle h, const double *z, uint64_t seed, uint32_t iter) {
   if (!h) return ST_ERR_USAGE;
-  invalidate_stats(h);
+  {
+    const bool live = h->seg_on && !h->comm && h->seg_valid && h->seg_phys == h->slot_map[0] && h->cache_gram && h->gram_valid;
+    invalidate_w(h);
+    h->seg_sweep = live;
+  }
   HCHK(h, hipSetDevice(h->device));
   int rc = gen_or_upload_z(h, z, seed, iter, 0u, h->d_z.p);
   if (rc) return rc;
@@ -2014,6 +2071,7 @@
   invalidate_stats(h);
   HCHK(h, hipSetDevice(h->device));
   const int rc = sample_launch(h, std::min(h->cut, h->n_actual_groups), 0);
+  h->seg_sweep = false;
   if (rc == ST_OK) h->gram_valid = true;
   return rc;
 }
@@ -2030,7 +2088,7 @@
 }
 extern "C" int st_mg_unpack_w(st_handle h) {
   if (!h) return ST_ERR_USAGE;
-  invalidate_stats(h);
+  invalidate_w(h);
   HCHK(h, hipSetDevice(h->device));
   double errw[64];
   HCHK(h, hipMemcpyAsync(h->d_w.p, h->d_tmp_n.p, (size_t)h->n_all * sizeof(double), hipMemcpyDeviceToDevice, h->stream));
@@ -2063,7 +2121,7 @@
 }
 extern "C" int st_mg_gather_w_unpack(st_handle h) {
   if (!h) return ST_ERR_USAGE;
-  invalidate_stats(h);
+  invalidate_w(h);
   HCHK(h, hipSetDevice(h->device));
   int rc = gather_w_scatter(h);
   if (rc) return rc;
@@ -2127,11 +2185,22 @@
       Gr.blks = h->d_blks.p; Gr.anc_idx = h->d_anc.p; Gr.grps = h->d_grps.p; Gr.list = h->d_owngrp.p; Gr.nlist = (int)h->own_grp_list.size();
       Gr.panels = h->d_panels[phys].p; Gr.w = h->d_w.p; Gr.loglik_c = h->d_loglik[phys].p; Gr.maxP = maxP;
       Gr.gdesc = h->d_gdesc.p; Gr.gd_stride = h->gd_stride;
-      hipLaunchKernelGGL(k_loglik_grp, dim3(Gr.nlist), dim3(NT), (size_t)(maxP + 32) * sizeof(double), h->stream, Gr);
+      const bool store = h->seg_on && !h->comm && phys == h->slot_map[0] && h->cache_gram && h->gram_valid;
+      Gr.segc = store ? h->d_seg.p : nullptr; Gr.segoff = store ? h->d_segoff.p : nullptr;
+      Gr.seg_ps = h->seg_ps;
+      const size_t stage = store ? (size_t)(NT / 64) * LOGLIK_SEG_RS * h->seg_ps : 0;
+      hipLaunchKernelGGL(k_loglik_grp, dim3(Gr.nlist), dim3(NT), ((size_t)maxP + 32 + stage) * sizeof(double), h->stream, Gr);
+      if (store) { h->seg_valid = true; h->seg_phys = phys; h->seg_stored += h->seg_levels; }
     }
   }
   HCHK(h, hipGetLastError());
   HCHK(h, reset_err(h) == ST_OK ? hipSuccess : hipErrorUnknown);
+  return ST_OK;
+}
+extern "C" int st_seg_handoff_counts(st_handle h, int64_t *stored, int64_t *used) {
+  if (!h) return ST_ERR_USAGE;
+  if (stored) *stored = h->seg_stored;
+  if (used) *used = h->seg_used;
   return ST_OK;
 }
 static int fix_top_comps(st_handle h, int phys) {
@@ -2170,7 +2239,7 @@
   (void)theta_changed;
   if (!h) return ST_ERR_USAGE;
   if (h->pred_list.empty()) return ST_OK;
-  invalidate_stats(h);
+  invalidate_w(h);
   if (!h->z_valid) { h->err = "st_predict needs the normals of a preceding st_sample_w (spamtree_model.cpp:1325)"; return ST_ERR_USAGE; }
   if (h->theta[0].empty()) { h->err = "st_predict before st_factor(slot 0)"; return ST_ERR_USAGE; }
   HCHK(h, hipSetDevice(h->device));
diff --git a/spamtree_amd/csrc/st_device.hpp b/spamtree_amd/csrc/st_device.hpp
--- a/spamtree_amd/csrc/st_device.hpp
+++ b/spamtree_amd/csrc/st_device.hpp
@@ -678,3 +678,11 @@
   if (s_coff && tid >= 128 && tid < 128 + H.ndch) s_coff[tid - 128] = s_gd[8 + 4 * H.nanc + 3 * H.nblk + (tid - 128)];
   return H;
 }
+
+
+__device__ __forceinline__ double seg_step(double a, double x, double w) { return __builtin_fma(x, w, a); }
+__device__ __forceinline__ double seg_walk(const double *x, const double *w, int ma) {
+  double a = 0.0;
+  for (int j = 0; j < ma; ++j) a = seg_step(a, x[j], w[j]);
+  return a;
+}
```

Measured after the change: 238.0. -1.3%, worse.
